# facebookresearch/D3GA

Hardware: AMD Instinct MI355X
Metric: fwd+bwd frames/sec @500k Gaussians 1920x1080 (higher is better)
Workload: dtype f32

## Files before the change

d3ga_amd/csrc/d3ga_internal.h:

```cpp
#pragma once
#include <hip/hip_runtime.h>
#include <stdint.h>

#include "../../include/d3ga.h"
#include "d3ga_math.h"

namespace d3ga {

constexpr int kBlock = 256;

int debug_knob(int key);

static inline int64_t align256(int64_t x) { return (x + 255) & ~int64_t(255); }

struct GeomBuf {
    float *depth;
    float4 *conic_o;
    float4 *rgb_invd;
    uint2 *rect;
    uint8_t *clamped;
    float *cov3D;
    float4 *xyh;
    float *dcol;
    int64_t dcol_stride;
};
static inline int64_t geom_bytes(int64_t P) {
    return align256(4 * P) + align256(16 * P) + align256(16 * P) + align256(8 * P) + align256(P) +
           align256(24 * P) + align256(16 * P) + align256(36 * P);
}
static inline GeomBuf carve_geom(void *base, int64_t P) {
    char *p = (char *)base;
    GeomBuf g;
    g.depth = (float *)p;     p += align256(4 * P);
    g.conic_o = (float4 *)p;  p += align256(16 * P);
    g.rgb_invd = (float4 *)p; p += align256(16 * P);
    g.rect = (uint2 *)p;      p += align256(8 * P);
    g.clamped = (uint8_t *)p; p += align256(P);
    g.cov3D = (float *)p;     p += align256(24 * P);
    g.xyh = (float4 *)p;      p += align256(16 * P);
    g.dcol = (float *)p;
    g.dcol_stride = P;
    return g;
}
__host__ __device__ static inline GeomBuf geom_view(const GeomBuf &g, int64_t P, int64_t v) {
    GeomBuf o = g;
    const int64_t d = v * P;
    o.depth += d; o.conic_o += d; o.rgb_invd += d; o.rect += d; o.clamped += d; o.cov3D += 6 * d; o.xyh += d; o.dcol += d;
    return o;
}

struct BinBuf {
    uint32_t *counters;
    uint32_t *tile_count;
    uint32_t *tile_start;
    uint32_t *tile_cursor;
    uint64_t *keys;
    uint32_t *point_list;
    uint32_t *big_tiles;
    uint32_t *huge_tiles;
    uint32_t *mid_tiles;
    uint32_t *tile_order;
};
static inline int64_t bin_bytes(int64_t tiles, int64_t dcap) {
    return 256 + align256(4 * tiles) + align256(4 * (tiles + 1)) + align256(4 * tiles) + align256(8 * dcap) +
           align256(4 * dcap) + 4 * align256(4 * tiles);
}
static inline BinBuf carve_bin(void *base, int64_t tiles, int64_t dcap) {
    char *p = (char *)base;
    BinBuf b;
    b.counters = (uint32_t *)p;    p += 256;
    b.tile_count = (uint32_t *)p;  p += align256(4 * tiles);
    b.tile_start = (uint32_t *)p;  p += align256(4 * (tiles + 1));
    b.tile_cursor = (uint32_t *)p; p += align256(4 * tiles);
    b.keys = (uint64_t *)p;        p += align256(8 * dcap);
    b.point_list = (uint32_t *)p;  p += align256(4 * dcap);
    b.big_tiles = (uint32_t *)p;   p += align256(4 * tiles);
    b.huge_tiles = (uint32_t *)p;  p += align256(4 * tiles);
    b.mid_tiles = (uint32_t *)p;   p += align256(4 * tiles);
    b.tile_order = (uint32_t *)p;
    return b;
}

struct ImgBuf {
    float *final_T;
    uint32_t *n_contrib;
    uint32_t *blk_count;
    uint2 *blk_list;
};
static inline int64_t img_bytes(int64_t W, int64_t H, int64_t tiles, int64_t dcap, int64_t views = 1) {
    return 2 * align256(4 * W * H * views) + align256(64 * tiles) + align256(128 * dcap);
}
static inline ImgBuf carve_img(void *base, int64_t W, int64_t H, int64_t tiles, int64_t views = 1) {
    ImgBuf i;
    char *p = (char *)base;
    i.final_T = (float *)p;        p += align256(4 * W * H * views);
    i.n_contrib = (uint32_t *)p;   p += align256(4 * W * H * views);
    i.blk_count = (uint32_t *)p;   p += align256(64 * tiles);
    i.blk_list = (uint2 *)p;
    return i;
}

constexpr int kWinTiles = 4096;

struct TileWindow {
    int x0, y0, w, h;
    __device__ __forceinline__ int area() const { return w * h; }
    __device__ __forceinline__ bool fits() const { return w * h <= kWinTiles; }
    __device__ __forceinline__ int tile_of(int k, int gx, float inv_w) const {
        const int r = (int)(((float)k + 0.5f) * inv_w);
        return (y0 + r) * gx + x0 + (k - r * w);
    }
};

#ifdef __HIPCC__
__device__ __forceinline__ TileWindow block_tile_window(int *s_box, bool visible, int rx0, int ry0, int rx1, int ry1) {
    if (threadIdx.x == 0) { s_box[0] = 0x7fffffff; s_box[1] = 0x7fffffff; s_box[2] = 0; s_box[3] = 0; }
    __syncthreads();
    int bx0 = visible ? rx0 : 0x7fffffff, by0 = visible ? ry0 : 0x7fffffff, bx1 = visible ? rx1 : 0, by1 = visible ? ry1 : 0;
#pragma unroll
    for (int off = 1; off < 64; off <<= 1) {
        bx0 = min(bx0, __shfl_xor(bx0, off)); by0 = min(by0, __shfl_xor(by0, off));
        bx1 = max(bx1, __shfl_xor(bx1, off)); by1 = max(by1, __shfl_xor(by1, off));
    }
    if ((threadIdx.x & 63) == 0 && bx1 > 0) {
        atomicMin(&s_box[0], bx0); atomicMin(&s_box[1], by0);
        atomicMax(&s_box[2], bx1); atomicMax(&s_box[3], by1);
    }
    __syncthreads();
    TileWindow win;
    win.x0 = s_box[0]; win.y0 = s_box[1];
    win.w = s_box[2] > s_box[0] ? s_box[2] - s_box[0] : 0;
    win.h = s_box[3] > s_box[1] ? s_box[3] - s_box[1] : 0;
    if (win.w == 0 || win.h == 0) { win.w = 0; win.h = 0; }
    return win;
}
#endif

static inline int tiles_x(int W) { return (W + kTile - 1) / kTile; }
static inline int tiles_y(int H) { return (H + kTile - 1) / kTile; }
static inline int n_views_of(const d3ga_raster_params *prm) { return prm->n_views > 1 ? prm->n_views : 1; }
static inline bool is_windowed(const d3ga_raster_params *prm) { return prm->tanfovx == D3GA_CAMERA_SLOT_WINDOWED; }
static inline int grid_x(const d3ga_raster_params *prm) { return tiles_x(prm->W) + (is_windowed(prm) ? 1 : 0); }
static inline int grid_y(const d3ga_raster_params *prm) { return tiles_y(prm->H) + (is_windowed(prm) ? 1 : 0); }
static inline int4 *win_table(void *binning, int64_t tiles, int64_t dcap) { return (int4 *)((char *)binning + bin_bytes(tiles, dcap)); }
static inline int64_t win_table_bytes(int64_t views) { return align256(16 * views); }

static inline int check_launch(hipStream_t s, int debug) {
    hipError_t e = hipGetLastError();
    if (e != hipSuccess) return (int)e;
    if (debug) {
        e = hipStreamSynchronize(s);
        if (e != hipSuccess) return (int)e;
    }
    return 0;
}

#define D3GA_TRY(expr)            \
    do {                          \
        int _st = (expr);         \
        if (_st != 0) return _st; \
    } while (0)
#define D3GA_HIP(expr)                          \
    do {                                        \
        hipError_t _e = (expr);                 \
        if (_e != hipSuccess) return (int)_e;   \
    } while (0)

#ifdef __HIPCC__
static __global__ void zero_words_kernel(uint32_t *__restrict__ p, size_t n) {
    for (size_t i = (size_t)blockIdx.x * blockDim.x + threadIdx.x; i < n; i += (size_t)gridDim.x * blockDim.x) p[i] = 0u;
}
static __global__ void zero_bytes_kernel(unsigned char *__restrict__ p, size_t n) {
    for (size_t i = (size_t)blockIdx.x * blockDim.x + threadIdx.x; i < n; i += (size_t)gridDim.x * blockDim.x) p[i] = 0;
}
static inline hipError_t zero_async(void *ptr, size_t bytes, hipStream_t s) {
    if (bytes == 0) return hipSuccess;
    if ((((uintptr_t)ptr | bytes) & 3) == 0) {
        const size_t n = bytes / 4;
        const size_t blocks = (n + 4 * kBlock - 1) / (4 * kBlock);
        hipLaunchKernelGGL(zero_words_kernel, dim3((unsigned)(blocks < 1 ? 1 : (blocks > 4096 ? 4096 : blocks))), dim3(kBlock), 0, s,
                           reinterpret_cast<uint32_t *>(ptr), n);
    } else {
        const size_t blocks = (bytes + kBlock - 1) / kBlock;
        hipLaunchKernelGGL(zero_bytes_kernel, dim3((unsigned)(blocks > 4096 ? 4096 : blocks)), dim3(kBlock), 0, s,
                           reinterpret_cast<unsigned char *>(ptr), bytes);
    }
    return hipGetLastError();
}
#endif

}
```

d3ga_amd/csrc/raster_api.hip:

```cpp
#include "d3ga_internal.h"

#include <atomic>

namespace d3ga {
static const int kKnobDefault[D3GA_KNOB_COUNT] = {
     32 | 128,  512,  2,  -1,  -1,
     1,  1,  0,  0};
static std::atomic<int> g_knob[D3GA_KNOB_COUNT] = {{32 | 128}, {512}, {2}, {-1}, {-1}, {1}, {1}, {0}, {0}};
int debug_knob(int key) { return (key >= 0 && key < D3GA_KNOB_COUNT) ? g_knob[key].load(std::memory_order_relaxed) : 0; }
}

using namespace d3ga;

extern "C" int d3ga_debug_set(int32_t key, int32_t value) {
    if (key < 0 || key >= D3GA_KNOB_COUNT) return D3GA_E_SIZE;
    g_knob[key].store(value == D3GA_KNOB_DEFAULT ? kKnobDefault[key] : value, std::memory_order_relaxed);
    return D3GA_OK;
}

extern "C" int d3ga_debug_defaults(int32_t *out, int32_t n) {
    if (!out) return D3GA_E_NULL;
    if (n < 2 + 2 * D3GA_KNOB_COUNT) return D3GA_E_SIZE;
#ifdef D3GA_SCAN_ABL
    out[0] = D3GA_SCAN_ABL;
#else
    out[0] = 0;
#endif
#ifdef D3GA_DIAG
    out[1] = 1;
#else
    out[1] = 0;
#endif
    for (int k = 0; k < D3GA_KNOB_COUNT; ++k) { out[2 + 2 * k] = kKnobDefault[k]; out[3 + 2 * k] = debug_knob(k); }
    return D3GA_OK;
}

extern "C" int d3ga_version(void) { return D3GA_VERSION; }

extern "C" const char *d3ga_status_string(int status) {
    switch (status) {
        case D3GA_OK: return "ok";
        case D3GA_E_NULL: return "required pointer is NULL";
        case D3GA_E_SIZE: return "negative or inconsistent size";
        case D3GA_E_CONFIG: return "unsupported argument combination";
        case D3GA_E_CAPACITY: return "scratch buffer too small";
        default: break;
    }
    if (status > 0) return hipGetErrorString((hipError_t)status);
    return "unknown status";
}

extern "C" int d3ga_raster_scratch_bytes_views(int32_t P, int32_t W, int32_t H, int32_t n_views, int64_t d_capacity,
                                               int32_t forward_only, int64_t sizes[3]) {
    if (!sizes) return D3GA_E_NULL;
    if (P < 0 || W <= 0 || H <= 0 || d_capacity < 0 || n_views < 0) return D3GA_E_SIZE;
    const int64_t k = n_views > 1 ? n_views : 1;
    if ((int64_t)tiles_y(H) * k > 65535 || (int64_t)P * k >= (1ll << 31)) return D3GA_E_SIZE;
    const int64_t tiles = (int64_t)tiles_x(W) * tiles_y(H) * k, cap = d_capacity > 0 ? d_capacity : 1;
    sizes[0] = geom_bytes(P > 0 ? P * k : 1);
    sizes[1] = bin_bytes(tiles, cap);
    sizes[2] = forward_only ? 2 * align256(4 * (int64_t)W * H * k) : img_bytes(W, H, tiles, cap, k);
    return D3GA_OK;
}

extern "C" int d3ga_raster_scratch_bytes_window(int32_t P, int32_t W, int32_t H, int32_t n_views, int64_t d_capacity,
                                                int32_t forward_only, int64_t sizes[3]) {
    if (!sizes) return D3GA_E_NULL;
    if (P < 0 || W <= 0 || H <= 0 || d_capacity < 0 || n_views < 0) return D3GA_E_SIZE;
    const int64_t k = n_views > 1 ? n_views : 1;
    const int64_t gx = tiles_x(W) + 1, gy = tiles_y(H) + 1;
    if (gy * k > 65535 || gx > 65535 || (int64_t)P * k >= (1ll << 31)) return D3GA_E_SIZE;
    const int64_t tiles = gx * gy * k, cap = d_capacity > 0 ? d_capacity : 1;
    sizes[0] = geom_bytes(P > 0 ? P * k : 1);
    sizes[1] = bin_bytes(tiles, cap) + win_table_bytes(k);
    sizes[2] = forward_only ? 2 * align256(4 * (int64_t)W * H * k) : img_bytes(W, H, tiles, cap, k);
    return D3GA_OK;
}

extern "C" int d3ga_raster_binning_layout_window(int32_t W, int32_t H, int32_t n_views, int64_t d_capacity, int64_t offsets[7]) {
    if (!offsets) return D3GA_E_NULL;
    if (W <= 0 || H <= 0 || d_capacity < 0 || n_views < 0) return D3GA_E_SIZE;
    const int64_t k = n_views > 1 ? n_views : 1, cap = d_capacity > 0 ? d_capacity : 1;
    const int64_t tiles = (int64_t)(tiles_x(W) + 1) * (tiles_y(H) + 1) * k;
    char *base = (char *)nullptr + 256;
    const BinBuf b = carve_bin(base, tiles, cap);
    offsets[0] = (char *)b.counters - base;
    offsets[1] = (char *)b.tile_count - base;
    offsets[2] = (char *)b.tile_start - base;
    offsets[3] = (char *)b.tile_cursor - base;
    offsets[4] = (char *)b.keys - base;
    offsets[5] = (char *)b.point_list - base;
    offsets[6] = (char *)win_table(base, tiles, cap) - base;
    return D3GA_OK;
}

extern "C" int d3ga_raster_scratch_bytes(int32_t P, int32_t W, int32_t H, int64_t d_capacity, int64_t sizes[3]) {
    return d3ga_raster_scratch_bytes_views(P, W, H, 1, d_capacity, 0, sizes);
}

extern "C" int64_t d3ga_raster_img_bytes(int32_t W, int32_t H, int64_t d_capacity, int32_t forward_only) {
    if (W <= 0 || H <= 0 || d_capacity < 0) return D3GA_E_SIZE;
    const int64_t tiles = (int64_t)tiles_x(W) * tiles_y(H);
    return forward_only ? 2 * align256(4 * (int64_t)W * H) : img_bytes(W, H, tiles, d_capacity > 0 ? d_capacity : 1);
}

extern "C" int d3ga_raster_binning_layout(int32_t W, int32_t H, int64_t d_capacity, int64_t offsets[6]) {
    if (!offsets) return D3GA_E_NULL;
    if (W <= 0 || H <= 0 || d_capacity < 0) return D3GA_E_SIZE;
    char *base = (char *)nullptr + 256;
    const BinBuf b = carve_bin(base, (int64_t)tiles_x(W) * tiles_y(H), d_capacity > 0 ? d_capacity : 1);
    offsets[0] = (char *)b.counters - base;
    offsets[1] = (char *)b.tile_count - base;
    offsets[2] = (char *)b.tile_start - base;
    offsets[3] = (char *)b.tile_cursor - base;
    offsets[4] = (char *)b.keys - base;
    offsets[5] = (char *)b.point_list - base;
    return D3GA_OK;
}

extern "C" int d3ga_raster_img_layout(int32_t W, int32_t H, int64_t offsets[2]) {
    if (!offsets) return D3GA_E_NULL;
    if (W <= 0 || H <= 0) return D3GA_E_SIZE;
    offsets[0] = 0;
    offsets[1] = align256(4 * (int64_t)W * H);
    return D3GA_OK;
}

extern "C" int d3ga_raster_img_layout_blocks(int32_t W, int32_t H, int64_t offsets[2]) {
    if (!offsets) return D3GA_E_NULL;
    if (W <= 0 || H <= 0) return D3GA_E_SIZE;
    const int64_t tiles = (int64_t)tiles_x(W) * tiles_y(H);
    char *base = (char *)nullptr + 256;
    const ImgBuf im = carve_img(base, W, H, tiles);
    offsets[0] = (char *)im.blk_count - base;
    offsets[1] = (char *)im.blk_list - base;
    return D3GA_OK;
}

extern "C" int d3ga_raster_forward(const d3ga_raster_params *prm, const float *means3D, const float *shs,
                                   const float *colors_precomp, const float *opacities, const float *scales,
                                   const float *rotations, const float *cov3D_precomp, const float *viewmatrix,
                                   const float *projmatrix, const float *campos, const float *bg, void *geom,
                                   void *binning, void *img, int64_t d_capacity, float *out_color, int32_t *radii,
                                   float *out_invdepth, d3ga_stream_t stream) {
    D3GA_TRY(d3ga_raster_preprocess(prm, means3D, shs, colors_precomp, opacities, scales, rotations, cov3D_precomp,
                                    viewmatrix, projmatrix, campos, geom, binning, d_capacity, radii, stream));
    D3GA_TRY(d3ga_raster_bin_sort(prm, geom, binning, d_capacity, stream));
    return d3ga_raster_composite_fwd(prm, bg, geom, binning, d_capacity, img, out_color, out_invdepth, stream);
}

extern "C" int d3ga_raster_backward(const d3ga_raster_params *prm, const float *means3D, const float *shs,
                                    const float *scales, const float *rotations, const float *cov3D_precomp,
                                    const float *viewmatrix, const float *projmatrix, const float *campos,
                                    const float *bg, const void *geom, const void *binning, int64_t d_capacity,
                                    const void *img, const float *dL_dpix, float *acc, float *dL_dmeans3D,
                                    float *dL_dmeans2D, float *dL_dopacity, float *dL_dsh, float *dL_dcolors,
                                    float *dL_dcov3D, float *dL_dscales, float *dL_drots, d3ga_stream_t stream) {
    if (prm && prm->P > 0 && acc && !prm->acc_self_clearing)
        D3GA_HIP(zero_async(acc, sizeof(float) * D3GA_ACC_STRIDE * (size_t)prm->P * (size_t)n_views_of(prm), (hipStream_t)stream));
    D3GA_TRY(d3ga_raster_composite_bwd(prm, bg, geom, binning, d_capacity, img, dL_dpix, acc, stream));
    return d3ga_raster_preprocess_bwd(prm, means3D, shs, scales, rotations, cov3D_precomp, viewmatrix, projmatrix,
                                      campos, geom, acc, dL_dmeans3D, dL_dmeans2D, dL_dopacity, dL_dsh, dL_dcolors,
                                      dL_dcov3D, dL_dscales, dL_drots, stream);
}

extern "C" int d3ga_raster_backward_l1(const d3ga_raster_params *prm, const float *means3D, const float *shs,
                                       const float *scales, const float *rotations, const float *cov3D_precomp,
                                       const float *viewmatrix, const float *projmatrix, const float *campos,
                                       const float *bg, const void *geom, const void *binning, int64_t d_capacity,
                                       const void *img, const float *image, const float *target, const void *target_cell,
                                       const float *g_loss, const float *dL_dpix, float *acc, float *dL_dmeans3D,
                                       float *dL_dmeans2D, float *dL_dopacity, float *dL_dsh, float *dL_dcolors,
                                       float *dL_dcov3D, float *dL_dscales, float *dL_drots, d3ga_stream_t stream) {
    if (prm && prm->P > 0 && acc && !prm->acc_self_clearing)
        D3GA_HIP(zero_async(acc, sizeof(float) * D3GA_ACC_STRIDE * (size_t)prm->P * (size_t)n_views_of(prm), (hipStream_t)stream));
    D3GA_TRY(d3ga_raster_composite_bwd_l1(prm, bg, geom, binning, d_capacity, img, image, target, target_cell, g_loss, dL_dpix,
                                          acc, stream));
    return d3ga_raster_preprocess_bwd(prm, means3D, shs, scales, rotations, cov3D_precomp, viewmatrix, projmatrix,
                                      campos, geom, acc, dL_dmeans3D, dL_dmeans2D, dL_dopacity, dL_dsh, dL_dcolors,
                                      dL_dcov3D, dL_dscales, dL_drots, stream);
}
```

d3ga_amd/csrc/raster_bin.hip:

```cpp
#include <atomic>

#include "composite_common.h"

namespace d3ga {

constexpr int kScanBlock = 1024;

__device__ __forceinline__ void tile_scan_body(int tiles, const uint32_t *__restrict__ count,
                                               uint32_t *__restrict__ start, uint32_t *__restrict__ cursor,
                                               uint32_t *__restrict__ counters, uint64_t dcap,
                                               uint32_t *__restrict__ big_tiles, uint32_t *__restrict__ huge_tiles,
                                               uint32_t *__restrict__ mid_tiles, uint32_t n_small, uint32_t n_mid,
                                               uint32_t n_large) {
    constexpr int kPer = 8, kChunk = kPer * kScanBlock;
    __shared__ uint32_t s_wave[2][kScanBlock / 64];
    __shared__ uint32_t s_max;
    const int tid = threadIdx.x, lane = tid & 63, wave = tid >> 6;
    if (tid == 0) s_max = 0;
    uint32_t carry = 0, mx = 0;
    int par = 0;
    for (int c0 = 0; c0 < tiles; c0 += kChunk, par ^= 1) {
        const int t0 = c0 + kPer * tid;
        uint32_t c[kPer];
        if (t0 + kPer <= tiles) {
            const uint4 lo = reinterpret_cast<const uint4 *>(count + t0)[0], hi = reinterpret_cast<const uint4 *>(count + t0)[1];
            c[0] = lo.x; c[1] = lo.y; c[2] = lo.z; c[3] = lo.w; c[4] = hi.x; c[5] = hi.y; c[6] = hi.z; c[7] = hi.w;
        } else {
#pragma unroll
            for (int k = 0; k < kPer; ++k) c[k] = t0 + k < tiles ? count[t0 + k] : 0u;
        }
        uint32_t sum = 0;
#pragma unroll
        for (int k = 0; k < kPer; ++k) { sum += c[k]; mx = max(mx, c[k]); }
        uint32_t incl = sum;
#pragma unroll
        for (int off = 1; off < 64; off <<= 1) {
            const uint32_t v = __shfl_up(incl, off);
            if (lane >= off) incl += v;
        }
        if (lane == 63) s_wave[par][wave] = incl;
        __syncthreads();
        uint32_t wbase = 0, total = 0;
#pragma unroll
        for (int w = 0; w < kScanBlock / 64; ++w) {
            const uint32_t v = s_wave[par][w];
            wbase += w < wave ? v : 0u;
            total += v;
        }
        uint32_t run = carry + wbase + incl - sum;
        uint32_t e[kPer];
        int cls[kPer];
#pragma unroll
        for (int k = 0; k < kPer; ++k) {
            e[k] = run;
            run += c[k];
            cls[k] = c[k] > n_large ? 2 : (c[k] > n_mid ? 1 : (c[k] > n_small ? 0 : -1));
        }
#pragma unroll
        for (int q = 0; q < 3; ++q) {
            uint32_t nq = 0;
#pragma unroll
            for (int k = 0; k < kPer; ++k) nq += cls[k] == q ? 1u : 0u;
            if (__ballot(nq != 0u) == 0ull) continue;
            uint32_t inq = nq;
#pragma unroll
            for (int off = 1; off < 64; off <<= 1) {
                const uint32_t v = __shfl_up(inq, off);
                if (lane >= off) inq += v;
            }
            const uint32_t tot = (uint32_t)__shfl((int)inq, 63);
            uint32_t base = 0;
            if (lane == 0) base = atomicAdd(&counters[q == 0 ? D3GA_CNT_MID : (q == 1 ? D3GA_CNT_BIG : D3GA_CNT_HUGE)], tot);
            uint32_t pos = (uint32_t)__shfl((int)base, 0) + inq - nq;
            uint32_t *list = q == 0 ? mid_tiles : (q == 1 ? big_tiles : huge_tiles);
#pragma unroll
            for (int k = 0; k < kPer; ++k)
                if (cls[k] == q) list[pos++] = (uint32_t)(t0 + k);
        }
        if (t0 + kPer <= tiles) {
            const uint4 lo = make_uint4(e[0], e[1], e[2], e[3]), hi = make_uint4(e[4], e[5], e[6], e[7]);
            reinterpret_cast<uint4 *>(start + t0)[0] = lo; reinterpret_cast<uint4 *>(start + t0)[1] = hi;
            reinterpret_cast<uint4 *>(cursor + t0)[0] = lo; reinterpret_cast<uint4 *>(cursor + t0)[1] = hi;
        } else {
#pragma unroll
            for (int k = 0; k < kPer; ++k)
                if (t0 + k < tiles) { start[t0 + k] = e[k]; cursor[t0 + k] = e[k]; }
        }
        carry += total;
    }
#pragma unroll
    for (int off = 1; off < 64; off <<= 1) mx = max(mx, (uint32_t)__shfl_xor((int)mx, off));
    if (lane == 0) atomicMax(&s_max, mx);
    __syncthreads();
    if (tid == 0) {
        start[tiles] = carry;
        counters[D3GA_CNT_D] = carry;
        counters[D3GA_CNT_OVERFLOW] = (uint64_t)carry > dcap ? 1u : 0u;
        counters[D3GA_CNT_MAXTILE] = s_max;
    }
}

__device__ __forceinline__ void tile_order_body(int tiles, const uint32_t *__restrict__ count,
                                                uint32_t *__restrict__ order, uint32_t *__restrict__ counters) {
    __shared__ uint32_t s_hist[256];
    __shared__ uint32_t s_zero;
    const int tid = threadIdx.x, lane = tid & 63;
    constexpr int kPer = 8;
    if (tid < 256) s_hist[tid] = 0;
    if (tid == 0) s_zero = 0;
    __syncthreads();
    auto bucket = [](uint32_t c) { return 254u - min(c >> 4, 254u); };
    for (int c0 = 0; c0 < tiles; c0 += kPer * kScanBlock) {
        uint32_t c[kPer];
#pragma unroll
        for (int k = 0; k < kPer; ++k) {
            const int t = c0 + k * kScanBlock + tid;
            c[k] = t < tiles ? count[t] : 0xffffffffu;
        }
#pragma unroll
        for (int k = 0; k < kPer; ++k) {
            const bool zero = c[k] == 0u;
            const unsigned long long zm = __ballot(zero);
            if (lane == 0 && zm) atomicAdd(&s_zero, (uint32_t)__popcll(zm));
            if (c[k] != 0u && c[k] != 0xffffffffu) atomicAdd(&s_hist[bucket(c[k])], 1u);
        }
        if (c0 + kPer * kScanBlock < tiles) continue;
        __syncthreads();
        if (tid < 64) {
            uint32_t v[4], sum = 0;
#pragma unroll
            for (int k = 0; k < 4; ++k) { v[k] = (4 * tid + k < 255) ? s_hist[4 * tid + k] : 0u; sum += v[k]; }
            uint32_t incl = sum;
#pragma unroll
            for (int off = 1; off < 64; off <<= 1) {
                const uint32_t u = __shfl_up(incl, off);
                if (tid >= off) incl += u;
            }
            uint32_t run = incl - sum;
#pragma unroll
            for (int k = 0; k < 4; ++k) { s_hist[4 * tid + k] = run; run += v[k]; }
        }
        __syncthreads();
        if (tid == 0) {
            s_zero = s_hist[255];
            counters[D3GA_CNT_HEAVY] = s_hist[255] <= 4096u ? (s_hist[255] + 9u) / 10u : 0u;
        }
        __syncthreads();
        for (int c1 = 0; c1 < tiles; c1 += kPer * kScanBlock) {
            if (c0 != 0) {
#pragma unroll
                for (int k = 0; k < kPer; ++k) {
                    const int t = c1 + k * kScanBlock + tid;
                    c[k] = t < tiles ? count[t] : 0xffffffffu;
                }
            }
#pragma unroll
            for (int k = 0; k < kPer; ++k) {
                const int t = c1 + k * kScanBlock + tid;
                const bool zero = c[k] == 0u;
                const unsigned long long zm = __ballot(zero);
                uint32_t zbase = 0;
                if (lane == 0 && zm) zbase = atomicAdd(&s_zero, (uint32_t)__popcll(zm));
                zbase = (uint32_t)__shfl((int)zbase, 0);
                if (zero) order[zbase + (uint32_t)__popcll(zm & ((1ull << lane) - 1ull))] = (uint32_t)t;
                if (c[k] != 0u && c[k] != 0xffffffffu) order[atomicAdd(&s_hist[bucket(c[k])], 1u)] = (uint32_t)t;
            }
        }
    }
}

__global__ __launch_bounds__(kScanBlock) void tile_scan_order_kernel(int tiles, const uint32_t *__restrict__ count,
                                                                     uint32_t *__restrict__ start,
                                                                     uint32_t *__restrict__ cursor,
                                                                     uint32_t *__restrict__ counters, uint64_t dcap,
                                                                     uint32_t *__restrict__ big_tiles,
                                                                     uint32_t *__restrict__ huge_tiles,
                                                                     uint32_t *__restrict__ mid_tiles, uint32_t n_small,
                                                                     uint32_t n_mid, uint32_t n_large,
                                                                     uint32_t *__restrict__ order) {
    if (blockIdx.x == 0) tile_scan_body(tiles, count, start, cursor, counters, dcap, big_tiles, huge_tiles, mid_tiles, n_small, n_mid, n_large);
    else tile_order_body(tiles, count, order, counters);
}

__global__ __launch_bounds__(kBlock) void tile_scatter_kernel(int P, int gx, const uint2 *__restrict__ rect,
                                                              const float *__restrict__ depth,
                                                              uint32_t *__restrict__ cursor, uint64_t *__restrict__ keys,
                                                              uint64_t dcap) {
    __shared__ int s_box[4];
    __shared__ uint32_t s_cnt[kWinTiles];
    const int tid = threadIdx.x;
    const int i = blockIdx.x * kBlock + tid;
    int x0 = 0, y0 = 0, x1 = 0, y1 = 0;
    uint64_t key = 0;
    if (i < P) {
        const uint2 rc = rect[i];
        x0 = rc.x & 0xffffu; y0 = rc.x >> 16; x1 = rc.y & 0xffffu; y1 = rc.y >> 16;
        key = ((uint64_t)__float_as_uint(depth[i]) << 32) | (uint32_t)i;
    }
    const bool visible = x1 > x0 && y1 > y0;
    const TileWindow win = block_tile_window(s_box, visible, x0, y0, x1, y1);
    const int area = win.area();
    if (area == 0) return;
    if (win.fits()) {
        for (int k = tid; k < area; k += kBlock) s_cnt[k] = 0;
        __syncthreads();
        if (visible)
            for (int ty = y0; ty < y1; ++ty)
                for (int tx = x0; tx < x1; ++tx) atomicAdd(&s_cnt[(ty - win.y0) * win.w + (tx - win.x0)], 1u);
        __syncthreads();
        const float inv_w = 1.0f / (float)win.w;
        for (int k = tid; k < area; k += kBlock) {
            const uint32_t c = s_cnt[k];
            if (c) s_cnt[k] = atomicAdd(&cursor[win.tile_of(k, gx, inv_w)], c);
        }
        __syncthreads();
        if (visible)
            for (int ty = y0; ty < y1; ++ty)
                for (int tx = x0; tx < x1; ++tx) {
                    const int l = (ty - win.y0) * win.w + (tx - win.x0);
                    const uint32_t pos = atomicAdd(&s_cnt[l], 1u);
                    if (pos < dcap) keys[pos] = key;
                }
    } else if (visible) {
        for (int ty = y0; ty < y1; ++ty)
            for (int tx = x0; tx < x1; ++tx) {
                const uint32_t pos = atomicAdd(&cursor[ty * gx + tx], 1u);
                if (pos < dcap) keys[pos] = key;
            }
    }
}

template <typename KeyPtr>
__device__ __forceinline__ void bitonic_sort(KeyPtr k, int n, int tid, int nthreads) {
    int n2 = 1;
    while (n2 < n) n2 <<= 1;
    const int half = n2 >> 1;
    for (int size = 2, lsz = 1; size <= n2; size <<= 1, ++lsz) {
        const int hs = size >> 1;
        for (int i = tid; i < half; i += nthreads) {
            const int blk = i >> (lsz - 1), off = i & (hs - 1);
            const int lo = (blk << lsz) + off, hi = (blk << lsz) + size - 1 - off;
            if (hi < n) {
                const uint64_t a = k[lo], b = k[hi];
                if (b < a) { k[lo] = b; k[hi] = a; }
            }
        }
        __syncthreads();
        for (int j = hs >> 1, lj = lsz - 2; j >= 1; j >>= 1, --lj) {
            for (int i = tid; i < half; i += nthreads) {
                const int blk = i >> lj, off = i & (j - 1);
                const int lo = (blk << (lj + 1)) + off, hi = lo + j;
                if (hi < n) {
                    const uint64_t a = k[lo], b = k[hi];
                    if (b < a) { k[lo] = b; k[hi] = a; }
                }
            }
            __syncthreads();
        }
    }
}

template <int BLOCK, int CAP>
__device__ __forceinline__ void sort_one_tile_bucket(uint64_t *s_key, uint32_t *s_bin, uint32_t *s_red, int tile,
                                                     const uint32_t *__restrict__ start, const uint64_t *__restrict__ keys,
                                                     uint32_t *__restrict__ point_list, uint64_t dcap) {
    static_assert(CAP == 8 * BLOCK, "eight keys / eight counters per thread");
    constexpr int NW = BLOCK / 64;
    const uint64_t b64 = min((uint64_t)start[tile], dcap), e64 = min((uint64_t)start[tile + 1], dcap);
    const int n = min((int)(e64 - b64), CAP);
    const int tid = threadIdx.x, lane = tid & 63, wave = tid >> 6;
    uint64_t r[8];
    uint32_t lo = 0xffffffffu, hi = 0u;
#pragma unroll
    for (int k = 0; k < 8; ++k) {
        const int i = tid + k * BLOCK;
        r[k] = i < n ? keys[b64 + i] : ~0ull;
    }
#pragma unroll
    for (int k = 0; k < 8; ++k) {
        const int i = tid + k * BLOCK;
        if (i < n) { const uint32_t d = (uint32_t)(r[k] >> 32); lo = min(lo, d); hi = max(hi, d); }
    }
#pragma unroll
    for (int off = 1; off < 64; off <<= 1) {
        lo = min(lo, (uint32_t)__shfl_xor((int)lo, off));
        hi = max(hi, (uint32_t)__shfl_xor((int)hi, off));
    }
    if (lane == 0) { s_red[wave] = lo; s_red[NW + wave] = hi; }
#pragma unroll
    for (int k = 0; k < 8; ++k) s_bin[tid + k * BLOCK] = 0u;
    __syncthreads();
#pragma unroll
    for (int w = 0; w < NW; ++w) { lo = min(lo, s_red[w]); hi = max(hi, s_red[NW + w]); }
    const uint32_t range = hi - lo;
    int sh = 32 - __clz((int)(range | 1u)) - (31 - __clz(CAP));
    if (range & 0x80000000u) sh = 32 - (31 - __clz(CAP));
    sh = max(sh, 0);
    uint32_t bucket[8], slot[8];
#pragma unroll
    for (int k = 0; k < 8; ++k) {
        const int i = tid + k * BLOCK;
        bucket[k] = ((uint32_t)(r[k] >> 32) - lo) >> sh;
        slot[k] = 0u;
        if (i < n) slot[k] = atomicAdd(&s_bin[bucket[k]], 1u);
    }
    __syncthreads();
    {
        uint32_t c[8], sum = 0;
#pragma unroll
        for (int k = 0; k < 8; ++k) { c[k] = s_bin[8 * tid + k]; sum += c[k]; }
        uint32_t incl = sum;
#pragma unroll
        for (int off = 1; off < 64; off <<= 1) {
            const uint32_t u = (uint32_t)__shfl_up((int)incl, off);
            if (lane >= off) incl += u;
        }
        if (lane == 63) s_red[wave] = incl;
        __syncthreads();
        uint32_t run = incl - sum;
#pragma unroll
        for (int w = 0; w < NW; ++w) if (w < wave) run += s_red[w];
#pragma unroll
        for (int k = 0; k < 8; ++k) { s_bin[8 * tid + k] = run; run += c[k]; }
        if (tid == BLOCK - 1) s_bin[CAP] = run;
    }
    __syncthreads();
#pragma unroll
    for (int k = 0; k < 8; ++k) {
        const int i = tid + k * BLOCK;
        if (i < n) s_key[s_bin[bucket[k]] + slot[k]] = r[k];
    }
    __syncthreads();
#pragma unroll
    for (int k = 0; k < 8; ++k) {
        const int i = tid + k * BLOCK;
        if (i < n) {
            const uint32_t b0 = s_bin[bucket[k]], b1 = s_bin[bucket[k] + 1];
            uint32_t less = 0;
            for (uint32_t p = b0; p < b1; ++p) less += s_key[p] < r[k] ? 1u : 0u;
            point_list[b64 + b0 + less] = (uint32_t)r[k];
        }
    }
}

template <int BLOCK, int CAP>
__device__ __forceinline__ bool sort_huge_tile_bucket(uint64_t *s_key, uint32_t *s_bin, uint32_t *s_cur, uint32_t *s_red, int tile,
                                                      const uint32_t *__restrict__ start, const uint64_t *__restrict__ keys,
                                                      uint32_t *__restrict__ point_list, uint64_t dcap) {
    static_assert(CAP == 8 * BLOCK, "eight counters per thread");
    constexpr int NW = BLOCK / 64;
    const uint64_t b64 = min((uint64_t)start[tile], dcap), e64 = min((uint64_t)start[tile + 1], dcap);
    const int n = (int)(e64 - b64);
    const int tid = threadIdx.x, lane = tid & 63, wave = tid >> 6;
    uint32_t lo = 0xffffffffu, hi = 0u;
    for (int i = tid; i < n; i += BLOCK) { const uint32_t d = (uint32_t)(keys[b64 + i] >> 32); lo = min(lo, d); hi = max(hi, d); }
#pragma unroll
    for (int off = 1; off < 64; off <<= 1) {
        lo = min(lo, (uint32_t)__shfl_xor((int)lo, off));
        hi = max(hi, (uint32_t)__shfl_xor((int)hi, off));
    }
    __syncthreads();
    if (lane == 0) { s_red[wave] = lo; s_red[NW + wave] = hi; }
#pragma unroll
    for (int k = 0; k < 8; ++k) s_bin[tid + k * BLOCK] = 0u;
    __syncthreads();
#pragma unroll
    for (int w = 0; w < NW; ++w) { lo = min(lo, s_red[w]); hi = max(hi, s_red[NW + w]); }
    const uint32_t range = hi - lo;
    const int sh = max(32 - __clz((int)(range | 1u)) - (31 - __clz(CAP)), 0);
    for (int i = tid; i < n; i += BLOCK) atomicAdd(&s_bin[((uint32_t)(keys[b64 + i] >> 32) - lo) >> sh], 1u);
    __syncthreads();
    uint32_t cmax = 0;
    {
        uint32_t c[8], sum = 0;
#pragma unroll
        for (int k = 0; k < 8; ++k) { c[k] = s_bin[8 * tid + k]; sum += c[k]; cmax = max(cmax, c[k]); }
        uint32_t incl = sum;
#pragma unroll
        for (int off = 1; off < 64; off <<= 1) {
            const uint32_t u = (uint32_t)__shfl_up((int)incl, off);
            if (lane >= off) incl += u;
            cmax = max(cmax, (uint32_t)__shfl_xor((int)cmax, off));
        }
        __syncthreads();
        if (lane == 63) { s_red[wave] = incl; s_red[NW + wave] = cmax; }
        __syncthreads();
        uint32_t run = incl - sum;
#pragma unroll
        for (int w = 0; w < NW; ++w) { if (w < wave) run += s_red[w]; cmax = max(cmax, s_red[NW + w]); }
#pragma unroll
        for (int k = 0; k < 8; ++k) { s_bin[8 * tid + k] = run; run += c[k]; }
        if (tid == BLOCK - 1) s_bin[CAP] = run;
    }
    __syncthreads();
    if (cmax > (uint32_t)CAP) return false;
    for (int segA = 0; segA < CAP;) {
        if (tid == 0) {
            const uint32_t limit = s_bin[segA] + (uint32_t)CAP;
            int a = segA + 1, b = CAP;
            while (a < b) { const int m = (a + b + 1) >> 1; if (s_bin[m] <= limit) a = m; else b = m - 1; }
            s_red[0] = (uint32_t)a;
        }
#pragma unroll
        for (int k = 0; k < 8; ++k) s_cur[tid + k * BLOCK] = 0u;
        __syncthreads();
        const int segB = (int)s_red[0];
        const uint32_t baseA = s_bin[segA], m = s_bin[segB] - baseA;
        if (m) {
            for (int i = tid; i < n; i += BLOCK) {
                const uint64_t key = keys[b64 + i];
                const uint32_t b = ((uint32_t)(key >> 32) - lo) >> sh;
                if (b >= (uint32_t)segA && b < (uint32_t)segB) s_key[s_bin[b] - baseA + atomicAdd(&s_cur[b], 1u)] = key;
            }
            __syncthreads();
            for (uint32_t i = tid; i < m; i += BLOCK) {
                const uint64_t key = s_key[i];
                const uint32_t b = ((uint32_t)(key >> 32) - lo) >> sh;
                const uint32_t b0 = s_bin[b] - baseA, b1 = s_bin[b + 1] - baseA;
                uint32_t less = 0;
                for (uint32_t p = b0; p < b1; ++p) less += s_key[p] < key ? 1u : 0u;
                point_list[b64 + baseA + b0 + less] = (uint32_t)key;
            }
        }
        __syncthreads();
        segA = segB;
    }
    return true;
}

template <int BLOCK, int CAP>
__global__ __launch_bounds__(BLOCK) void tile_sort_lds_kernel(const uint32_t *__restrict__ start,
                                                              const uint64_t *__restrict__ keys,
                                                              uint32_t *__restrict__ point_list, uint64_t dcap,
                                                              const uint32_t *__restrict__ order, int tiles) {
    __shared__ uint64_t s_key[CAP];
    __shared__ __attribute__((aligned(8))) uint32_t s_bin[CAP + 1];
    __shared__ uint32_t s_red[2 * (BLOCK / 64)];
    for (int rank = blockIdx.x; rank < tiles; rank += gridDim.x) {
        const int tile = (int)order[rank];
        const uint32_t n = start[tile + 1] - start[tile];
        if (n == 0) return;
        if (n <= (uint32_t)CAP) sort_one_tile_bucket<BLOCK, CAP>(s_key, s_bin, s_red, tile, start, keys, point_list, dcap);
        __syncthreads();
    }
}

template <int BLOCK, int CAP>
__global__ __launch_bounds__(BLOCK) void tile_sort_lds_list_kernel(const uint32_t *__restrict__ start,
                                                                   const uint64_t *__restrict__ keys,
                                                                   uint32_t *__restrict__ point_list, uint64_t dcap,
                                                                   const uint32_t *__restrict__ list,
                                                                   const uint32_t *__restrict__ list_count,
                                                                   uint64_t *__restrict__ keys_rw,
                                                                   const uint32_t *__restrict__ huge_list,
                                                                   const uint32_t *__restrict__ huge_count,
                                                                   const uint32_t *__restrict__ list2,
                                                                   const uint32_t *__restrict__ list2_count) {
    extern __shared__ __attribute__((aligned(16))) uint64_t s_key_dyn[];
    uint32_t *s_bin = reinterpret_cast<uint32_t *>(s_key_dyn + CAP);
    uint32_t *s_red = s_bin + CAP + 1;
    uint32_t *s_cur = s_red + 2 * (BLOCK / 64) + 2;
    const uint32_t count = *list_count;
    for (uint32_t v = blockIdx.x; v < count; v += gridDim.x) {
        __syncthreads();
        sort_one_tile_bucket<BLOCK, CAP>(s_key_dyn, s_bin, s_red, (int)list[v], start, keys, point_list, dcap);
    }
    if (list2) {
        const uint32_t count2 = *list2_count;
        for (uint32_t v = gridDim.x - 1u - blockIdx.x; v < count2; v += gridDim.x) {
            __syncthreads();
            sort_one_tile_bucket<BLOCK, CAP>(s_key_dyn, s_bin, s_red, (int)list2[v], start, keys, point_list, dcap);
        }
    }
    if (huge_list) {
        const uint32_t hcount = *huge_count;
        const int tid = threadIdx.x;
        for (uint32_t k = blockIdx.x; k < hcount; k += gridDim.x) {
            const int tile = (int)huge_list[k];
            const uint64_t b64 = min((uint64_t)start[tile], dcap), e64 = min((uint64_t)start[tile + 1], dcap);
            const int n = (int)(e64 - b64);
            __syncthreads();
            if (!sort_huge_tile_bucket<BLOCK, CAP>(s_key_dyn, s_bin, s_cur, s_red, tile, start, keys, point_list, dcap)) {
                bitonic_sort(keys_rw + b64, n, tid, BLOCK);
                for (int i = tid; i < n; i += BLOCK) point_list[b64 + i] = (uint32_t)keys_rw[b64 + i];
            }
        }
    }
}

}

using namespace d3ga;

constexpr int kSortSmall = 2048;
constexpr int kSortMid = 4096;
constexpr int kSortLarge = 8192;
static inline size_t sort_lds_bytes(int cap, int block, bool huge = false) {
    return (size_t)cap * 8 + ((size_t)cap + 1 + 2 * (block / 64) + 2 + (huge ? cap : 0)) * 4 + 16;
}


extern "C" int d3ga_raster_bin_sort(const d3ga_raster_params *prm, void *geom, void *binning, int64_t d_capacity,
                                    d3ga_stream_t stream) {
    if (!prm || !geom || !binning) return D3GA_E_NULL;
    if (prm->P < 0 || prm->W <= 0 || prm->H <= 0 || d_capacity < 0) return D3GA_E_SIZE;
    hipStream_t s = (hipStream_t)stream;
    const int views = n_views_of(prm);
    const int gx = grid_x(prm);
    const int tiles = gx * grid_y(prm) * views;
    const int64_t P = (int64_t)prm->P * views;
    BinBuf bin = carve_bin(binning, tiles, d_capacity);
    GeomBuf g = carve_geom(geom, P);
    hipLaunchKernelGGL(tile_scan_order_kernel, dim3(2), dim3(kScanBlock), 0, s, tiles, bin.tile_count, bin.tile_start,
                       bin.tile_cursor, bin.counters, (uint64_t)d_capacity, bin.big_tiles, bin.huge_tiles, bin.mid_tiles,
                       (uint32_t)kSortSmall, (uint32_t)kSortMid, (uint32_t)kSortLarge, bin.tile_order);
    D3GA_TRY(check_launch(s, prm->debug));
    if (P == 0 || d_capacity == 0) return D3GA_OK;
    hipLaunchKernelGGL(tile_scatter_kernel, dim3((unsigned)((P + kBlock - 1) / kBlock)), dim3(kBlock), 0, s, (int)P, gx, g.rect,
                       g.depth, bin.tile_cursor, bin.keys, (uint64_t)d_capacity);
    D3GA_TRY(check_launch(s, prm->debug));
    {
        static std::atomic<int> resident[64] = {};
        int dev = 0;
        D3GA_HIP(hipGetDevice(&dev));
        int want = (dev >= 0 && dev < 64) ? resident[dev].load(std::memory_order_relaxed) : 0;
        if (want == 0) {
            int per_cu = 0, cus = 0;
            if (hipOccupancyMaxActiveBlocksPerMultiprocessor(&per_cu, (const void *)tile_sort_lds_kernel<256, kSortSmall>, 256, 0) != hipSuccess || per_cu < 1) per_cu = 4;
            if (hipDeviceGetAttribute(&cus, hipDeviceAttributeMultiprocessorCount, dev) != hipSuccess || cus < 1) cus = 256;
            want = per_cu * cus;
            if (dev >= 0 && dev < 64) resident[dev].store(want, std::memory_order_relaxed);
        }
        hipLaunchKernelGGL((tile_sort_lds_kernel<256, kSortSmall>), dim3(tiles < want ? tiles : want), dim3(256), 0, s, bin.tile_start,
                           bin.keys, bin.point_list, (uint64_t)d_capacity, (const uint32_t *)bin.tile_order, tiles);
    }
    D3GA_TRY(check_launch(s, prm->debug));
    {
        static std::atomic<bool> attr_set[64] = {};
        int dev = 0;
        D3GA_HIP(hipGetDevice(&dev));
        if (dev >= 0 && dev < 64 && !attr_set[dev].load(std::memory_order_relaxed)) {
            D3GA_HIP(hipFuncSetAttribute((const void *)tile_sort_lds_list_kernel<1024, kSortLarge>,
                                         hipFuncAttributeMaxDynamicSharedMemorySize, (int)sort_lds_bytes(kSortLarge, 1024, true)));
            attr_set[dev].store(true, std::memory_order_relaxed);
        }
    }
    const int lgrid = tiles < 256 ? tiles : 256, mgrid = tiles < 768 ? tiles : 768;
    const int merge_knob = debug_knob(D3GA_KNOB_SORT_MERGE);
    const bool merged = merge_knob >= 0 ? merge_knob != 0 : d_capacity / (tiles > 0 ? tiles : 1) < 320;
#define D3GA_LAUNCH_LIST_SORT(BLOCKV, CAPV, GRID, HUGE, LIST, CNT, KEYS_RW, HLIST, HCNT, LIST2, CNT2)                              \
    hipLaunchKernelGGL((tile_sort_lds_list_kernel<BLOCKV, CAPV>), dim3(GRID), dim3(BLOCKV), sort_lds_bytes(CAPV, BLOCKV, HUGE), s, \
                       bin.tile_start, bin.keys, bin.point_list, (uint64_t)d_capacity, LIST, CNT, KEYS_RW, HLIST, HCNT, LIST2, CNT2)
    const uint32_t *const nil = nullptr;
    if (!merged) {
        D3GA_LAUNCH_LIST_SORT(512, kSortMid, mgrid, false, bin.mid_tiles, bin.counters + D3GA_CNT_MID, (uint64_t *)nullptr, nil, nil, nil, nil);
        D3GA_TRY(check_launch(s, prm->debug));
    }
    const uint32_t *l2 = merged ? (const uint32_t *)bin.mid_tiles : nil, *c2 = merged ? (const uint32_t *)(bin.counters + D3GA_CNT_MID) : nil;
    D3GA_LAUNCH_LIST_SORT(1024, kSortLarge, lgrid, true, bin.big_tiles, bin.counters + D3GA_CNT_BIG, bin.keys,
                          (const uint32_t *)bin.huge_tiles, (const uint32_t *)(bin.counters + D3GA_CNT_HUGE), l2, c2);
#undef D3GA_LAUNCH_LIST_SORT
    return check_launch(s, prm->debug);
}
```

d3ga_amd/csrc/raster_pre.hip:

```cpp
#include "composite_common.h"
#include "raster_pre_body.h"

namespace d3ga {

constexpr int kShRow = 52;
constexpr int kShSlab = 64 * kShRow;
constexpr size_t kShLdsBytes = (size_t)(kBlock / 64) * kShSlab * sizeof(float);

__host__ __device__ __forceinline__ bool sh_staged(int M) { return M > 0 && (3 * M) % 4 == 0 && 3 * M <= 48; }

__device__ __forceinline__ void sh_slab_load(float *slab, const float *__restrict__ src, int rows, int M3, int lane) {
    const int nvec = rows * M3 / 4;
    for (int v = lane; v < nvec; v += 64) {
        const float4 x = reinterpret_cast<const float4 *>(src)[v];
        const int e = 4 * v, r = e / M3, c = e - r * M3;
        *reinterpret_cast<float4 *>(slab + r * kShRow + c) = x;
    }
}
__device__ __forceinline__ void sh_slab_store(const float *slab, float *__restrict__ dst, int rows, int M3, int lane) {
    const int nvec = rows * M3 / 4;
    for (int v = lane; v < nvec; v += 64) {
        const int e = 4 * v, r = e / M3, c = e - r * M3;
        reinterpret_cast<float4 *>(dst)[v] = *reinterpret_cast<const float4 *>(slab + r * kShRow + c);
    }
}

template <int ROWS>
struct ShRegs { float4 v[ROWS * 12 / 64]; };
template <int ROWS>
__device__ __forceinline__ ShRegs<ROWS> sh_rows48_load(const float *__restrict__ src, int lane) {
    ShRegs<ROWS> r;
#pragma unroll
    for (int k = 0; k < ROWS * 12 / 64; ++k) r.v[k] = reinterpret_cast<const float4 *>(src)[lane + 64 * k];
    return r;
}
template <int ROWS>
__device__ __forceinline__ void sh_rows48_to_slab(float *slab, const ShRegs<ROWS> &r, int lane) {
#pragma unroll
    for (int k = 0; k < ROWS * 12 / 64; ++k) {
        const int e = 4 * (lane + 64 * k), row = e / 48, c = e - row * 48;
        *reinterpret_cast<float4 *>(slab + row * kShRow + c) = r.v[k];
    }
}
template <int ROWS>
__device__ __forceinline__ void sh_rows48_store(const float *slab, float *__restrict__ dst, int lane) {
#pragma unroll
    for (int k = 0; k < ROWS * 12 / 64; ++k) {
        const int e = 4 * (lane + 64 * k), row = e / 48, c = e - row * 48;
        reinterpret_cast<float4 *>(dst)[lane + 64 * k] = *reinterpret_cast<const float4 *>(slab + row * kShRow + c);
    }
}

constexpr int kShPassRows = 32;
constexpr int kShHalfSlab = kShPassRows * kShRow;
constexpr size_t kShHalfLdsBytes = (size_t)(kBlock / 64) * kShHalfSlab * sizeof(float);

template <bool WANT_J>
__device__ __forceinline__ void staged_sh_colour(const d3ga_raster_params &prm, const float *__restrict__ means3D,
                                                 const float *__restrict__ shs, const float *__restrict__ campos,
                                                 float *s_sh, float acc[3], ShColJ &cj) {
    const int tid = threadIdx.x, lane = tid & 63, wave = tid >> 6;
    const int i = blockIdx.x * kBlock + tid;
    const int M3 = 3 * prm.M;
    float *slab = s_sh + wave * kShHalfSlab;
    const int row0 = blockIdx.x * kBlock + wave * 64;
    const int rows = min(64, prm.P - row0);
    const int nb = (prm.sh_degree + 1) * (prm.sh_degree + 1);
    float B[16];
    float dx = 0.f, dy = 0.f, dz = 1.f;
    if (WANT_J && i < prm.P) sh_view_dir(means3D, i, campos, dx, dy, dz);
    auto eval = [&](const float *row) __attribute__((always_inline)) {
        if (WANT_J) cj = sh_accumulate_jacobian(B, dx, dy, dz, row, nb, cj);
        else sh_accumulate(B, row, 0, 16, nb, acc);
    };
    if (M3 == 48 && rows == 64) {
        const float *src = shs + (size_t)48 * row0;
        const ShRegs<kShPassRows> h0 = sh_rows48_load<kShPassRows>(src, lane);
        const ShRegs<kShPassRows> h1 = sh_rows48_load<kShPassRows>(src + 48 * kShPassRows, lane);
        sh_view_basis(prm, means3D, i, campos, B);
        __builtin_amdgcn_wave_barrier();
        sh_rows48_to_slab<kShPassRows>(slab, h0, lane);
        __builtin_amdgcn_wave_barrier();
        if (lane / kShPassRows == 0) eval(slab + (lane % kShPassRows) * kShRow);
        __builtin_amdgcn_wave_barrier();
        sh_rows48_to_slab<kShPassRows>(slab, h1, lane);
        __builtin_amdgcn_wave_barrier();
        if (lane / kShPassRows == 1) eval(slab + (lane % kShPassRows) * kShRow);
        return;
    }
    if (i < prm.P) sh_view_basis(prm, means3D, i, campos, B);
    for (int h = 0; h < 2; ++h) {
        const int r = min(kShPassRows, rows - kShPassRows * h);
        __builtin_amdgcn_wave_barrier();
        if (r > 0) sh_slab_load(slab, shs + (size_t)M3 * (row0 + kShPassRows * h), r, M3, lane);
        __builtin_amdgcn_wave_barrier();
        if (i < prm.P && lane / kShPassRows == h) eval(slab + (lane % kShPassRows) * kShRow);
    }
}

struct TileRect { bool visible; int r0, r1, r2, r3; };
__device__ __forceinline__ TileRect write_geom_records(const GeomBuf &geom, int i, const PreOut &o, bool keep_cov, int tile_row0,
                                                       int32_t *__restrict__ radii, bool want_j, const ShColJ &cj) {
    const Splat &sp = o.sp;
    if (keep_cov) {
#pragma unroll
        for (int k = 0; k < 6; ++k) geom.cov3D[6 * (size_t)i + k] = o.c6[k];
    }
    radii[i] = sp.radius;
    geom.depth[i] = sp.depth;
    geom.rect[i] = sp.visible ? make_uint2((uint32_t)sp.rect[0] | ((uint32_t)(sp.rect[1] + tile_row0) << 16),
                                           (uint32_t)sp.rect[2] | ((uint32_t)(sp.rect[3] + tile_row0) << 16))
                              : make_uint2(0u, 0u);
    geom.conic_o[i] = make_float4(sp.conic[0], sp.conic[1], sp.conic[2], o.opacity);
    {
        const SplatCull sc = splat_cull(sp.conic[0], sp.conic[1], sp.conic[2], o.opacity);
        geom.xyh[i] = make_float4(sp.px, sp.py, sp.visible ? sc.hx : -1.0f, sc.hy);
    }
    geom.rgb_invd[i] = make_float4(o.rgb[0], o.rgb[1], o.rgb[2], sp.visible ? 1.0f / sp.depth : 0.f);
    geom.clamped[i] = o.clampmask;
    if (want_j) dcol_store(geom.dcol, geom.dcol_stride, i, cj);
    return TileRect{sp.visible, sp.rect[0], sp.rect[1] + tile_row0, sp.rect[2], sp.rect[3] + tile_row0};
}

__device__ __forceinline__ PreOut window_clip(PreOut o, int x0, int y0, int gx, int gy) {
    Splat &sp = o.sp;
    const int r0 = max(sp.rect[0], x0) - x0, r1 = max(sp.rect[1], y0) - y0;
    const int r2 = min(sp.rect[2], x0 + gx) - x0, r3 = min(sp.rect[3], y0 + gy) - y0;
    if (sp.visible && r2 > r0 && r3 > r1) { sp.rect[0] = r0; sp.rect[1] = r1; sp.rect[2] = r2; sp.rect[3] = r3; }
    else { sp.visible = false; sp.rect[0] = sp.rect[1] = sp.rect[2] = sp.rect[3] = 0; }
    return o;
}
__global__ void window_table_kernel(d3ga_raster_params prm, const float *__restrict__ campos, int views, int4 *__restrict__ table) {
    const int v = blockIdx.x * blockDim.x + threadIdx.x;
    if (v >= views) return;
    const ViewCam c = view_cam(prm, nullptr, nullptr, campos + (size_t)D3GA_CAMERA_SLOT_WINDOWED_FLOATS * v, true);
    table[v] = make_int4(c.ox, c.oy, c.W, c.H);
}

__device__ __forceinline__ void tile_histogram(int *s_box, uint32_t *s_cnt, const TileRect &t, int gx, uint32_t *__restrict__ tile_count,
                                               uint32_t *__restrict__ counters) {
    const int tid = threadIdx.x;
    const TileWindow win = block_tile_window(s_box, t.visible, t.r0, t.r1, t.r2, t.r3);
    const int nvis = __syncthreads_count(t.visible);
    if (tid == 0 && nvis) atomicAdd(&counters[D3GA_CNT_VISIBLE], (uint32_t)nvis);
    const int area = win.area();
    if (area == 0) return;
    if (win.fits()) {
        for (int k = tid; k < area; k += kBlock) s_cnt[k] = 0;
        __syncthreads();
        if (t.visible)
            for (int ty = t.r1; ty < t.r3; ++ty)
                for (int tx = t.r0; tx < t.r2; ++tx) atomicAdd(&s_cnt[(ty - win.y0) * win.w + (tx - win.x0)], 1u);
        __syncthreads();
        const float inv_w = 1.0f / (float)win.w;
        for (int k = tid; k < area; k += kBlock) {
            const uint32_t c = s_cnt[k];
            if (c) atomicAdd(&tile_count[win.tile_of(k, gx, inv_w)], c);
        }
    } else if (t.visible) {
        for (int ty = t.r1; ty < t.r3; ++ty)
            for (int tx = t.r0; tx < t.r2; ++tx) atomicAdd(&tile_count[ty * gx + tx], 1u);
    }
}

template <bool WIN>
__device__ __forceinline__ TileRect preprocess_view(const d3ga_raster_params &prm, const ViewCam &cam, int i, const float *means3D,
                                                    const float *sh_row, bool staged, const ShColJ &cj, bool pre, const float (&pc6)[6],
                                                    float pop, const float *colors_precomp, const float *opacities, const float *scales,
                                                    const float *rotations, const float *cov3D_precomp, const GeomBuf &geom,
                                                    int tile_row0, int32_t *radii, bool want_j, int gx, int gy) {
    PreLoaded pl;
    pl.has_sh = staged; pl.has_c6 = pre;
    pl.sh[0] = cj.a0; pl.sh[1] = cj.a1; pl.sh[2] = cj.a2;
#pragma unroll
    for (int k = 0; k < 6; ++k) pl.c6[k] = pc6[k];
    pl.op = pop;
    PreOut o = preprocess_one(prm, cam, i, means3D, sh_row, colors_precomp, opacities, scales, rotations, cov3D_precomp, pl);
    if constexpr (WIN) o = window_clip(o, cam.ox / kTile, cam.oy / kTile, gx, gy);
    return write_geom_records(geom, i, o, !cov3D_precomp, tile_row0, radii, want_j, cj);
}

template <bool WANT_J, bool WIN>
__global__ __launch_bounds__(kBlock) void preprocess_kernel(
    d3ga_raster_params prm, const float *__restrict__ means3D, const float *__restrict__ shs,
    const float *__restrict__ colors_precomp, const float *__restrict__ opacities, const float *__restrict__ scales,
    const float *__restrict__ rotations, const float *__restrict__ cov3D_precomp, const float *__restrict__ viewmatrix,
    const float *__restrict__ projmatrix, const float *__restrict__ campos, GeomBuf geom,
    uint32_t *__restrict__ tile_count, uint32_t *__restrict__ counters, int32_t *__restrict__ radii,
    int tile_row0 ) {
    const ViewCam cam = view_cam(prm, viewmatrix, projmatrix, campos, WIN);
    const int gx = (prm.W + kTile - 1) / kTile + (WIN ? 1 : 0), gy = (prm.H + kTile - 1) / kTile + 1;
    extern __shared__ __attribute__((aligned(16))) char smem[];
    __shared__ int s_box[4];
    float *s_sh = reinterpret_cast<float *>(smem);
    uint32_t *s_cnt = reinterpret_cast<uint32_t *>(smem);
    const int tid = threadIdx.x;
    const int i = blockIdx.x * kBlock + tid;
    const int M3 = 3 * prm.M;
    const bool staged = shs != nullptr && sh_staged(prm.M);
    float pc6[6] = {0.f, 0.f, 0.f, 0.f, 0.f, 0.f}, pop = 0.f;
    const bool pre = staged && cov3D_precomp != nullptr;
    if (pre && i < prm.P) {
#pragma unroll
        for (int k = 0; k < 6; ++k) pc6[k] = cov3D_precomp[6 * (size_t)i + k];
        pop = opacities[i];
    }
    ShColJ cj = {0.f, 0.f, 0.f, 0.f, 0.f, 0.f, 0.f, 0.f, 0.f, 0.f, 0.f, 0.f};
    float acc[3] = {0.f, 0.f, 0.f};
    if (staged) {
        staged_sh_colour<WANT_J>(prm, means3D, shs, campos, s_sh, acc, cj);
        if (!WANT_J) { cj.a0 = acc[0]; cj.a1 = acc[1]; cj.a2 = acc[2]; }
        __syncthreads();
    }
    TileRect tr = {false, 0, 0, 0, 0};
    if (i < prm.P) {
        tr = staged ? preprocess_view<WIN>(prm, cam, i, means3D, nullptr, true, cj, pre, pc6, pop, colors_precomp, opacities, scales,
                                           rotations, cov3D_precomp, geom, tile_row0, radii, WANT_J, gx, gy)
                    : preprocess_view<WIN>(prm, cam, i, means3D, shs ? shs + (size_t)M3 * i : nullptr, false, cj, false, pc6, pop,
                                           colors_precomp, opacities, scales, rotations, cov3D_precomp, geom, tile_row0, radii,
                                           WANT_J, gx, gy);
    }
    tile_histogram(s_box, s_cnt, tr, gx, tile_count, counters);
}

template <bool WANT_J, int KV>
__device__ __forceinline__ void staged_sh_colour_views(const d3ga_raster_params &prm, const float *__restrict__ means3D, size_t pv,
                                                       const float *__restrict__ shs, const ViewCams<KV> &cams, float *s_sh,
                                                       ShColJ (&cj)[KV]) {
    const int tid = threadIdx.x, lane = tid & 63, wave = tid >> 6;
    const int i = blockIdx.x * kBlock + tid;
    const int M3 = 3 * prm.M;
    float *slab = s_sh + wave * kShHalfSlab;
    const int row0 = blockIdx.x * kBlock + wave * 64;
    const int rows = min(64, prm.P - row0);
    const int nb = (prm.sh_degree + 1) * (prm.sh_degree + 1);
    auto eval = [&](const float *row) __attribute__((always_inline)) {
#pragma unroll
        for (int v = 0; v < KV; ++v) {
            float B[16];
            const float *mv = means3D + 3 * pv * v;
            if (WANT_J) {
                float dx, dy, dz;
                sh_view_dir(mv, i, cams.cp[v], dx, dy, dz);
                sh_basis(prm.sh_degree, dx, dy, dz, B);
                cj[v] = sh_accumulate_jacobian(B, dx, dy, dz, row, nb, cj[v]);
            } else {
                sh_view_basis(prm, mv, i, cams.cp[v], B);
                float acc[3] = {cj[v].a0, cj[v].a1, cj[v].a2};
                sh_accumulate(B, row, 0, 16, nb, acc);
                cj[v].a0 = acc[0]; cj[v].a1 = acc[1]; cj[v].a2 = acc[2];
            }
        }
    };
    if (M3 == 48 && rows == 64) {
        const float *src = shs + (size_t)48 * row0;
        const ShRegs<kShPassRows> h0 = sh_rows48_load<kShPassRows>(src, lane);
        const ShRegs<kShPassRows> h1 = sh_rows48_load<kShPassRows>(src + 48 * kShPassRows, lane);
        __builtin_amdgcn_wave_barrier();
        sh_rows48_to_slab<kShPassRows>(slab, h0, lane);
        __builtin_amdgcn_wave_barrier();
        if (lane / kShPassRows == 0) eval(slab + (lane % kShPassRows) * kShRow);
        __builtin_amdgcn_wave_barrier();
        sh_rows48_to_slab<kShPassRows>(slab, h1, lane);
        __builtin_amdgcn_wave_barrier();
        if (lane / kShPassRows == 1) eval(slab + (lane % kShPassRows) * kShRow);
        return;
    }
    for (int h = 0; h < 2; ++h) {
        const int r = min(kShPassRows, rows - kShPassRows * h);
        __builtin_amdgcn_wave_barrier();
        if (r > 0) sh_slab_load(slab, shs + (size_t)M3 * (row0 + kShPassRows * h), r, M3, lane);
        __builtin_amdgcn_wave_barrier();
        if (i < prm.P && lane / kShPassRows == h) eval(slab + (lane % kShPassRows) * kShRow);
    }
}

template <bool WANT_J, int KV>
__global__ __launch_bounds__(kBlock) void preprocess_views_kernel(
    d3ga_raster_params prm, const float *__restrict__ means3D, const float *__restrict__ shs,
    const float *__restrict__ colors_precomp, const float *__restrict__ opacities, const float *__restrict__ scales,
    const float *__restrict__ rotations, const float *__restrict__ cov3D_precomp, ViewCams<KV> cams, GeomBuf geom ,
    uint32_t *__restrict__ tile_count, uint32_t *__restrict__ counters, int32_t *__restrict__ radii ,
    int tile_row0, int gyv, size_t pv ) {
    extern __shared__ __attribute__((aligned(16))) char smem[];
    __shared__ int s_box[4];
    float *s_sh = reinterpret_cast<float *>(smem);
    uint32_t *s_cnt = reinterpret_cast<uint32_t *>(smem);
    const int tid = threadIdx.x;
    const int i = blockIdx.x * kBlock + tid;
    float pc6[6] = {0.f, 0.f, 0.f, 0.f, 0.f, 0.f}, pop = 0.f;
    const bool pre = cov3D_precomp != nullptr && pv == 0;
    if (pre && i < prm.P) {
#pragma unroll
        for (int k = 0; k < 6; ++k) pc6[k] = cov3D_precomp[6 * (size_t)i + k];
        pop = opacities[i];
    }
    ShColJ cj[KV];
#pragma unroll
    for (int v = 0; v < KV; ++v) cj[v] = ShColJ{0.f, 0.f, 0.f, 0.f, 0.f, 0.f, 0.f, 0.f, 0.f, 0.f, 0.f, 0.f};
    staged_sh_colour_views<WANT_J, KV>(prm, means3D, pv, shs, cams, s_sh, cj);
    const int gx = (prm.W + kTile - 1) / kTile;
#pragma unroll
    for (int v = 0; v < KV; ++v) {
        __syncthreads();
        TileRect tr = {false, 0, 0, 0, 0};
        if (i < prm.P) {
            const size_t og = pv * v;
            tr = preprocess_view<false>(prm, view_cam(prm, cams.vm[v], cams.pm[v], cams.cp[v], false), i, means3D + 3 * og, nullptr, true,
                                        cj[v], pre, pc6, pop, colors_precomp, opacities, scales ? scales + 3 * og : nullptr,
                                        rotations ? rotations + 4 * og : nullptr, cov3D_precomp ? cov3D_precomp + 6 * og : nullptr,
                                        geom_view(geom, prm.P, v), tile_row0 + v * gyv, radii + (size_t)prm.P * v, WANT_J, gx, 0);
        }
        tile_histogram(s_box, s_cnt, tr, gx, tile_count, counters);
    }
}

template <bool WANT_J>
__global__ __launch_bounds__(kBlock) void recolor_kernel(d3ga_raster_params prm, const float *__restrict__ means3D,
                                                         const float *__restrict__ shs,
                                                         const float *__restrict__ colors_precomp,
                                                         const float *__restrict__ campos, GeomBuf src, GeomBuf dst) {
    extern __shared__ __attribute__((aligned(16))) char smem[];
    float *s_sh = reinterpret_cast<float *>(smem);
    const int i = blockIdx.x * kBlock + threadIdx.x;
    const int M3 = 3 * prm.M;
    const bool staged = shs != nullptr && sh_staged(prm.M);
    ShColJ cj = {0.f, 0.f, 0.f, 0.f, 0.f, 0.f, 0.f, 0.f, 0.f, 0.f, 0.f, 0.f};
    float acc[3] = {0.f, 0.f, 0.f};
    if (staged) staged_sh_colour<WANT_J>(prm, means3D, shs, campos, s_sh, acc, cj);
    if (i >= prm.P) return;
    if (WANT_J) {
        acc[0] = cj.a0; acc[1] = cj.a1; acc[2] = cj.a2;
        dcol_store(dst.dcol, dst.dcol_stride, i, cj);
    }
    const uint2 rc = src.rect[i];
    const bool visible = rect_visible(rc.x, rc.y);
    const float depth = src.depth[i];
    dst.depth[i] = depth;
    dst.conic_o[i] = src.conic_o[i];
    dst.xyh[i] = src.xyh[i];
    dst.rect[i] = rc;
#pragma unroll
    for (int k = 0; k < 6; ++k) dst.cov3D[6 * (size_t)i + k] = src.cov3D[6 * (size_t)i + k];
    float rgb[3] = {0.f, 0.f, 0.f};
    uint8_t mask = 0;
    if (visible) {
        if (colors_precomp) {
            rgb[0] = colors_precomp[3 * (size_t)i]; rgb[1] = colors_precomp[3 * (size_t)i + 1];
            rgb[2] = colors_precomp[3 * (size_t)i + 2];
        } else {
            if (!staged) {
                float B[16];
                sh_view_basis(prm, means3D, i, campos, B);
                sh_accumulate(B, shs + (size_t)M3 * i, 0, 16, (prm.sh_degree + 1) * (prm.sh_degree + 1), acc);
            }
#pragma unroll
            for (int c = 0; c < 3; ++c) {
                const float v = acc[c] + 0.5f;
                if (v < 0.f) mask |= (uint8_t)(1u << c);
                rgb[c] = fmaxf(v, 0.f);
            }
        }
    }
    dst.rgb_invd[i] = make_float4(rgb[0], rgb[1], rgb[2], visible ? 1.0f / depth : 0.f);
    dst.clamped[i] = mask;
}

__device__ __forceinline__ ViewRecs view_recs(const GeomBuf &g, const float *acc) {
    return ViewRecs{reinterpret_cast<const uint32_t *>(g.rect), acc, g.clamped, reinterpret_cast<const float *>(g.conic_o), g.dcol,
                    g.dcol_stride};
}

template <bool WIN>
__global__ __launch_bounds__(kBlock) void preprocess_bwd_kernel(
    d3ga_raster_params prm, const float *__restrict__ means3D, const float *__restrict__ shs,
    const float *__restrict__ scales, const float *__restrict__ rotations, const float *__restrict__ viewmatrix,
    const float *__restrict__ projmatrix, const float *__restrict__ campos, GeomBuf geom,
    const float *__restrict__ acc, float *__restrict__ dL_dmeans3D, float *__restrict__ dL_dmeans2D,
    float *__restrict__ dL_dopacity, float *__restrict__ dL_dsh, float *__restrict__ dL_dcolors,
    float *__restrict__ dL_dcov3D, float *__restrict__ dL_dscales, float *__restrict__ dL_drots,
    const float *__restrict__ cov3D_precomp, int accum ) {
    const ViewCam cam = view_cam(prm, viewmatrix, projmatrix, campos, WIN);
    extern __shared__ __attribute__((aligned(16))) char smem[];
    float *s_sh = reinterpret_cast<float *>(smem);
    const int tid = threadIdx.x, lane = tid & 63, wave = tid >> 6;
    const int i = blockIdx.x * kBlock + tid;
    const int M3 = 3 * prm.M;
    const bool staged = shs != nullptr && sh_staged(prm.M);
    const int row0 = blockIdx.x * kBlock + wave * 64;
    const int rows = min(64, prm.P - row0);
    float *slab = s_sh + wave * kShSlab;
    const bool full48 = M3 == 48 && rows == 64;
    uint2 rc = make_uint2(0u, 0u);
    AccRec ar;
    float c6[6] = {0.f, 0.f, 0.f, 0.f, 0.f, 0.f};
    uint8_t clampmask = 0;
    float act_opacity = 0.f;
    if (i < prm.P) {
        rc = geom.rect[i];
        ar = acc_load(acc, i, prm.acc_self_clearing);
#pragma unroll
        for (int k = 0; k < 6; ++k) c6[k] = (cov3D_precomp ? cov3D_precomp : geom.cov3D)[6 * (size_t)i + k];
        clampmask = geom.clamped[i];
        act_opacity = geom.conic_o[i].w;
    }
    const bool have_j = staged && !prm.forward_only;
    ShColJ jd = {0.f, 0.f, 0.f, 0.f, 0.f, 0.f, 0.f, 0.f, 0.f, 0.f, 0.f, 0.f};
    if (have_j && i < prm.P) jd = dcol_load(geom.dcol, geom.dcol_stride, i);
    if (staged && !have_j) {
        if (full48) sh_rows48_to_slab<64>(slab, sh_rows48_load<64>(shs + (size_t)48 * row0, lane), lane);
        else if (rows > 0) sh_slab_load(slab, shs + (size_t)M3 * row0, rows, M3, lane);
        __builtin_amdgcn_wave_barrier();
    }
    if (i < prm.P) {
        const bool visible = rect_visible(rc.x, rc.y);
        if (!visible) {
#pragma unroll
            for (int k = 0; k < 12; ++k) ar.a[k] = 0.f;
#pragma unroll
            for (int k = 0; k < 6; ++k) c6[k] = 0.f;
            act_opacity = 0.f;
        }
        if (staged)
            preprocess_bwd_one(prm, cam, i, visible, means3D, slab + lane * kShRow, scales, rotations, c6, clampmask, ar.a, dL_dmeans3D,
                               dL_dmeans2D, dL_dopacity, dL_dsh ? slab + lane * kShRow : nullptr, dL_dcolors, dL_dcov3D, dL_dscales,
                               dL_drots, act_opacity, have_j, jd, accum);
        else
            preprocess_bwd_one(prm, cam, i, visible, means3D, shs ? shs + (size_t)M3 * i : nullptr, scales, rotations, c6, clampmask,
                               ar.a, dL_dmeans3D, dL_dmeans2D, dL_dopacity, dL_dsh ? dL_dsh + (size_t)M3 * i : nullptr, dL_dcolors,
                               dL_dcov3D, dL_dscales, dL_drots, act_opacity, false, ShColJ(), accum);
    }
    if (staged && dL_dsh) {
        __builtin_amdgcn_wave_barrier();
        if (full48) sh_rows48_store<64>(slab, dL_dsh + (size_t)48 * row0, lane);
        else if (rows > 0) sh_slab_store(slab, dL_dsh + (size_t)M3 * row0, rows, M3, lane);
    }
}

constexpr int kMaxGroup = 8;
template <bool WIN>
__global__ __launch_bounds__(kBlock) void preprocess_bwd_views_kernel(
    d3ga_raster_params prm, int kv, const float *__restrict__ means3D, bool sh_path, const float *__restrict__ scales,
    const float *__restrict__ rotations, const float *__restrict__ cov3D_precomp, ViewCams<kMaxGroup> cams, GeomBuf geom ,
    const float *__restrict__ acc , float *__restrict__ dL_dmeans3D, float *__restrict__ dL_dmeans2D ,
    float *__restrict__ dL_dopacity, float *__restrict__ dL_dsh, float *__restrict__ dL_dcolors, float *__restrict__ dL_dcov3D,
    float *__restrict__ dL_dscales, float *__restrict__ dL_drots, bool accum,
    size_t pv ,
    bool pva ) {
    extern __shared__ __attribute__((aligned(16))) char smem[];
    float *s_sh = reinterpret_cast<float *>(smem);
    const int tid = threadIdx.x, lane = tid & 63, wave = tid >> 6;
    const int i = blockIdx.x * kBlock + tid;
    const int M3 = 3 * prm.M;
    const int row0 = blockIdx.x * kBlock + wave * 64;
    const int rows = min(64, prm.P - row0);
    float *slab = s_sh + wave * kShSlab;
    if (i < prm.P)
        preprocess_bwd_views_one(prm, i, kv, WIN, cams, view_recs(geom, acc), means3D, cov3D_precomp ? cov3D_precomp : geom.cov3D,
                                 scales, rotations, sh_path, pv, pva, accum, dL_dmeans3D, dL_dmeans2D, dL_dopacity, dL_dcolors,
                                 dL_dcov3D, dL_dscales, dL_drots, sh_path && dL_dsh ? slab + lane * kShRow : nullptr);
    if (sh_path && dL_dsh) {
        __builtin_amdgcn_wave_barrier();
        if (accum) {
            const int nvec = rows > 0 ? rows * M3 / 4 : 0;
            float4 *dst = reinterpret_cast<float4 *>(dL_dsh + (size_t)M3 * row0);
            for (int v = lane; v < nvec; v += 64) {
                const int e = 4 * v, r = e / M3, c = e - r * M3;
                const float4 x = *reinterpret_cast<const float4 *>(slab + r * kShRow + c);
                float4 y = dst[v];
                y.x += x.x; y.y += x.y; y.z += x.z; y.w += x.w;
                dst[v] = y;
            }
        } else if (M3 == 48 && rows == 64) sh_rows48_store<64>(slab, dL_dsh + (size_t)48 * row0, lane);
        else if (rows > 0) sh_slab_store(slab, dL_dsh + (size_t)M3 * row0, rows, M3, lane);
    }
}

__global__ __launch_bounds__(kBlock) void sh_grad_from_views_kernel(
    int P, int M, int sh_degree, int n_views, const float *__restrict__ means3D, int64_t means_stride ,
    const float *__restrict__ g_views, int64_t g_stride, const float *__restrict__ campos_views, int64_t campos_stride, float scale,
    float *__restrict__ dL_dsh) {
    extern __shared__ __attribute__((aligned(16))) char smem[];
    float *s_sh = reinterpret_cast<float *>(smem);
    const int tid = threadIdx.x, lane = tid & 63, wave = tid >> 6;
    const int i = blockIdx.x * kBlock + tid;
    const int M3 = 3 * M;
    const bool staged = sh_staged(M);
    const int row0 = blockIdx.x * kBlock + wave * 64;
    const int rows = min(64, P - row0);
    float *slab = s_sh + wave * kShSlab;
    if (i < P) {
        float out[48];
#pragma unroll
        for (int k = 0; k < 48; ++k) out[k] = 0.f;
        const int nb = (sh_degree + 1) * (sh_degree + 1);
        for (int v = 0; v < n_views; ++v) {
            const float *g = g_views + v * g_stride + 3 * (size_t)i;
            const float g0 = g[0], g1 = g[1], g2 = g[2];
            if (g0 == 0.f && g1 == 0.f && g2 == 0.f) continue;
            const V3 mean = ld3(means3D + v * means_stride, i);
            const float *cp = campos_views + v * campos_stride;
            const V3 d0 = mean - v3(cp[0], cp[1], cp[2]);
            const float inv = 1.0f / sqrtf(dot(d0, d0));
            float B[16];
            sh_basis(sh_degree, d0.x * inv, d0.y * inv, d0.z * inv, B);
#pragma unroll
            for (int k = 0; k < 16; ++k)
                if (k < nb) {
                    out[3 * k] += B[k] * g0; out[3 * k + 1] += B[k] * g1; out[3 * k + 2] += B[k] * g2;
                }
        }
        float *row = staged ? slab + lane * kShRow : nullptr;
#pragma unroll
        for (int k = 0; k < 48; ++k)
            if (k < M3) {
                if (staged) row[k] = out[k] * scale;
                else dL_dsh[(size_t)M3 * i + k] = out[k] * scale;
            }
    }
    if (staged) {
        __syncthreads();
        if (rows > 0) sh_slab_store(slab, dL_dsh + (size_t)M3 * row0, rows, M3, lane);
    }
}

__global__ __launch_bounds__(kBlock) void mark_visible_kernel(int P, const float *__restrict__ means3D,
                                                              const float *__restrict__ viewmatrix,
                                                              uint8_t *__restrict__ visible) {
    const int i = blockIdx.x * kBlock + threadIdx.x;
    if (i >= P) return;
    visible[i] = xform_point(viewmatrix, ld3(means3D, i)).z > kNear ? 1 : 0;
}

}

using namespace d3ga;

static int validate(const d3ga_raster_params *prm) {
    if (!prm) return D3GA_E_NULL;
    if (prm->P < 0 || prm->W <= 0 || prm->H <= 0 || prm->M < 0 || prm->M > 16) return D3GA_E_SIZE;
    if (prm->sh_degree < 0 || prm->sh_degree > 3) return D3GA_E_CONFIG;
    if (prm->n_views < 0) return D3GA_E_SIZE;
    if (grid_x(prm) > 65535 || (int64_t)grid_y(prm) * n_views_of(prm) > 65535) return D3GA_E_SIZE;
    if ((int64_t)prm->P * n_views_of(prm) >= (1ll << 31)) return D3GA_E_SIZE;
    return D3GA_OK;
}

static bool staged(const d3ga_raster_params *prm, const float *shs) { return shs != nullptr && sh_staged(prm->M); }
static bool leaves_dcol(const d3ga_raster_params *prm, const float *shs) { return staged(prm, shs) && !prm->forward_only; }
static size_t lds_bytes(bool staged, size_t slabs, size_t floor = 0) { return staged && slabs > floor ? slabs : floor; }
static int cam_stride(const d3ga_raster_params *prm) {
    return prm->tanfovx > 0.f ? 3 : (is_windowed(prm) ? D3GA_CAMERA_SLOT_WINDOWED_FLOATS : 5);
}
template <int K>
static ViewCams<K> view_cams(const float *vm, const float *pm, const float *cp, int stride, int v0, int kv) {
    ViewCams<K> c;
    for (int q = 0; q < K; ++q) {
        const int v = v0 + (q < kv ? q : 0);
        c.vm[q] = vm + 16 * (size_t)v; c.pm[q] = pm + 16 * (size_t)v; c.cp[q] = cp + (size_t)stride * v;
    }
    return c;
}
template <class T>
static T *at(T *p, size_t n, size_t r) { return p ? p + n * r : nullptr; }

extern "C" int d3ga_raster_preprocess(const d3ga_raster_params *prm, const float *means3D, const float *shs,
                                      const float *colors_precomp, const float *opacities, const float *scales,
                                      const float *rotations, const float *cov3D_precomp, const float *viewmatrix,
                                      const float *projmatrix, const float *campos, void *geom, void *binning,
                                      int64_t d_capacity, int32_t *radii, d3ga_stream_t stream) {
    D3GA_TRY(validate(prm));
    if (!geom || !binning || !viewmatrix || !projmatrix || !campos) return D3GA_E_NULL;
    if (d_capacity < 0) return D3GA_E_SIZE;
    hipStream_t s = (hipStream_t)stream;
    const int views = n_views_of(prm), gyv = grid_y(prm);
    const int64_t tiles = (int64_t)grid_x(prm) * gyv * views;
    const bool wnd = is_windowed(prm);
    BinBuf bin = carve_bin(binning, tiles, d_capacity);
    D3GA_HIP(zero_async(bin.counters, 256 + align256(4 * tiles), s));
    if (wnd) hipLaunchKernelGGL(window_table_kernel, dim3((views + 63) / 64), dim3(64), 0, s, *prm, campos, views, win_table(binning, tiles, d_capacity));
    if (prm->P == 0) return D3GA_OK;
    if ((shs != nullptr) == (colors_precomp != nullptr)) return D3GA_E_CONFIG;
    const bool pva = views > 1 && prm->per_view_appearance;
    if (pva && shs) return D3GA_E_CONFIG;
    const bool sr = scales != nullptr && rotations != nullptr;
    if (sr == (cov3D_precomp != nullptr)) return D3GA_E_CONFIG;
    if (shs && (prm->sh_degree + 1) * (prm->sh_degree + 1) > prm->M) return D3GA_E_CONFIG;
    if (!means3D || !opacities || !radii) return D3GA_E_NULL;
    const GeomBuf g = carve_geom(geom, (int64_t)prm->P * views);
    const size_t lds = lds_bytes(staged(prm, shs), kShHalfLdsBytes, (size_t)kWinTiles * 4);
    const bool want_j = leaves_dcol(prm, shs);
    const int cs = cam_stride(prm);
    const size_t pv = (views > 1 && prm->per_view_geometry) ? (size_t)prm->P : 0;
    const size_t pa = pva ? (size_t)prm->P : 0;
    const dim3 grid((prm->P + kBlock - 1) / kBlock), block(kBlock);
    int v0 = 0;
    const bool grouped = views > 1 && !pva && !wnd && staged(prm, shs);
    auto launch_group = [&](auto kv) {
        constexpr int KV = decltype(kv)::value;
        const size_t og = pv * v0;
        hipLaunchKernelGGL((want_j ? preprocess_views_kernel<true, KV> : preprocess_views_kernel<false, KV>), grid, block, lds, s, *prm,
                           at(means3D, 3, og), shs, colors_precomp, opacities, at(scales, 3, og), at(rotations, 4, og),
                           at(cov3D_precomp, 6, og), view_cams<KV>(viewmatrix, projmatrix, campos, cs, v0, KV), geom_view(g, prm->P, v0),
                           bin.tile_count, bin.counters, radii + (size_t)prm->P * v0, v0 * gyv, gyv, pv);
        v0 += KV;
    };
    while (grouped && views - v0 >= 2) {
        const int left = views - v0;
        if (left >= 4 && left != 5) launch_group(std::integral_constant<int, 4>());
        else if (left == 3 || left == 5) launch_group(std::integral_constant<int, 3>());
        else launch_group(std::integral_constant<int, 2>());
    }
    const auto kernel = want_j ? (wnd ? preprocess_kernel<true, true> : preprocess_kernel<true, false>)
                               : (wnd ? preprocess_kernel<false, true> : preprocess_kernel<false, false>);
    for (int v = v0; v < views; ++v) {
        const ViewCams<1> c = view_cams<1>(viewmatrix, projmatrix, campos, cs, v, 1);
        const size_t og = pv * v, oa = pa * v;
        hipLaunchKernelGGL(kernel, grid, block, lds, s, *prm, at(means3D, 3, og), shs, at(colors_precomp, 3, oa), opacities + oa,
                           at(scales, 3, og), at(rotations, 4, og), at(cov3D_precomp, 6, og), c.vm[0], c.pm[0], c.cp[0],
                           geom_view(g, prm->P, v), bin.tile_count, bin.counters, radii + (size_t)prm->P * v, v * gyv);
    }
    return check_launch(s, prm->debug & 0xff);
}

extern "C" int d3ga_raster_recolor(const d3ga_raster_params *prm, const float *means3D, const float *shs,
                                   const float *colors_precomp, const float *campos, const void *geom_src,
                                   void *geom_dst, d3ga_stream_t stream) {
    D3GA_TRY(validate(prm));
    if (n_views_of(prm) > 1 || is_windowed(prm)) return D3GA_E_CONFIG;
    if (prm->P == 0) return D3GA_OK;
    if (!geom_src || !geom_dst || geom_src == geom_dst) return D3GA_E_NULL;
    if ((shs != nullptr) == (colors_precomp != nullptr)) return D3GA_E_CONFIG;
    if (shs && (!means3D || !campos)) return D3GA_E_NULL;
    if (shs && (prm->sh_degree + 1) * (prm->sh_degree + 1) > prm->M) return D3GA_E_CONFIG;
    hipStream_t s = (hipStream_t)stream;
    const GeomBuf src = carve_geom(const_cast<void *>(geom_src), prm->P), dst = carve_geom(geom_dst, prm->P);
    hipLaunchKernelGGL(leaves_dcol(prm, shs) ? recolor_kernel<true> : recolor_kernel<false>, dim3((prm->P + kBlock - 1) / kBlock),
                       dim3(kBlock), lds_bytes(staged(prm, shs), kShHalfLdsBytes), s, *prm, means3D, shs, colors_precomp, campos, src, dst);
    return check_launch(s, prm->debug & 0xff);
}

extern "C" int d3ga_raster_preprocess_bwd(const d3ga_raster_params *prm, const float *means3D, const float *shs,
                                          const float *scales, const float *rotations, const float *cov3D_precomp,
                                          const float *viewmatrix, const float *projmatrix, const float *campos,
                                          const void *geom, const float *acc, float *dL_dmeans3D, float *dL_dmeans2D,
                                          float *dL_dopacity, float *dL_dsh, float *dL_dcolors, float *dL_dcov3D,
                                          float *dL_dscales, float *dL_drots, d3ga_stream_t stream) {
    D3GA_TRY(validate(prm));
    if (prm->P == 0) return D3GA_OK;
    if (!means3D || !viewmatrix || !projmatrix || !campos || !geom || !acc || !dL_dmeans3D) return D3GA_E_NULL;
    if (dL_dsh && !shs) return D3GA_E_NULL;
    if (shs && !dL_dsh && !dL_dcolors) return D3GA_E_NULL;
    if ((dL_dscales != nullptr) != (dL_drots != nullptr)) return D3GA_E_CONFIG;
    if (dL_dscales && (!scales || !rotations)) return D3GA_E_NULL;
    if (!cov3D_precomp && !(scales && rotations)) return D3GA_E_NULL;
    hipStream_t s = (hipStream_t)stream;
    const int views = n_views_of(prm);
    const bool pva = views > 1 && prm->per_view_appearance;
    if (pva && shs) return D3GA_E_CONFIG;
    const GeomBuf g = carve_geom(const_cast<void *>(geom), (int64_t)prm->P * views);
    const size_t lds = lds_bytes(staged(prm, shs), kShLdsBytes);
    const bool win = is_windowed(prm);
    const int cs = cam_stride(prm);
    const dim3 grid((prm->P + kBlock - 1) / kBlock), block(kBlock);
    const size_t pv = prm->per_view_geometry ? (size_t)prm->P : 0;
    auto launch_view = [&](int v, float *dsh, float *dcol, int accum) {
        const ViewCams<1> c = view_cams<1>(viewmatrix, projmatrix, campos, cs, v, 1);
        const size_t o = (size_t)prm->P * v, og = pv * v;
        hipLaunchKernelGGL(win ? preprocess_bwd_kernel<true> : preprocess_bwd_kernel<false>, grid, block, lds, s, *prm, at(means3D, 3, og),
                           shs, at(scales, 3, og), at(rotations, 4, og), c.vm[0], c.pm[0], c.cp[0], geom_view(g, prm->P, v),
                           acc + D3GA_ACC_STRIDE * o, dL_dmeans3D + 3 * og, at(dL_dmeans2D, 3, o), dL_dopacity, dsh, dcol,
                           at(dL_dcov3D, 6, og), at(dL_dscales, 3, og), at(dL_drots, 4, og), at(cov3D_precomp, 6, og), accum);
    };
    if (views == 1) {
        launch_view(0, dL_dsh, dL_dcolors, 0);
        return check_launch(s, prm->debug);
    }
    if (shs ? (dL_dsh != nullptr && leaves_dcol(prm, shs)) : true) {
        for (int v0 = 0; v0 < views; v0 += kMaxGroup) {
            const int kv = views - v0 < kMaxGroup ? views - v0 : kMaxGroup;
            const size_t o = (size_t)prm->P * v0, og = pv * v0, oa = pva ? o : 0;
            hipLaunchKernelGGL(win ? preprocess_bwd_views_kernel<true> : preprocess_bwd_views_kernel<false>, grid, block, lds, s, *prm, kv,
                               at(means3D, 3, og), shs != nullptr, at(scales, 3, og), at(rotations, 4, og), at(cov3D_precomp, 6, og),
                               view_cams<kMaxGroup>(viewmatrix, projmatrix, campos, cs, v0, kv), geom_view(g, prm->P, v0),
                               acc + D3GA_ACC_STRIDE * o, dL_dmeans3D + 3 * og, at(dL_dmeans2D, 3, o), at(dL_dopacity, 1, oa), dL_dsh,
                               at(dL_dcolors, 3, oa), at(dL_dcov3D, 6, og), at(dL_dscales, 3, og), at(dL_drots, 4, og), v0 > 0, pv, pva);
        }
        return check_launch(s, prm->debug);
    }
    if (pva) return D3GA_E_CONFIG;
    if (shs && !dL_dcolors) return D3GA_E_NULL;
    if (prm->factor_rows != 0 && prm->factor_rows < prm->P) return D3GA_E_SIZE;
    const size_t fr = prm->factor_rows > 0 ? (size_t)prm->factor_rows : (size_t)prm->P;
    for (int v = 0; v < views; ++v) launch_view(v, nullptr, shs ? dL_dcolors + 3 * fr * v : dL_dcolors, v > 0 ? (pv ? 1 : 3) : 0);
    D3GA_TRY(check_launch(s, prm->debug));
    if (shs && dL_dsh) {
        hipLaunchKernelGGL(sh_grad_from_views_kernel, grid, block, lds_bytes(sh_staged(prm->M), kShLdsBytes), s, prm->P, prm->M,
                           prm->sh_degree, views, means3D, (int64_t)(3 * pv), dL_dcolors, (int64_t)(3 * fr), campos, (int64_t)cs, 1.0f, dL_dsh);
        return check_launch(s, prm->debug);
    }
    return D3GA_OK;
}

extern "C" int d3ga_sh_grad_from_views(int32_t P, int32_t M, int32_t sh_degree, int32_t n_views, const float *means3D,
                                       const float *g_views, int64_t g_stride, const float *campos_views,
                                       int64_t campos_stride, float scale, float *dL_dsh, d3ga_stream_t stream) {
    if (P < 0 || M < 1 || M > 16 || n_views < 0) return D3GA_E_SIZE;
    if (sh_degree < 0 || sh_degree > 3 || (sh_degree + 1) * (sh_degree + 1) > M) return D3GA_E_CONFIG;
    if (P == 0) return D3GA_OK;
    if (!means3D || !dL_dsh || (n_views > 0 && (!g_views || !campos_views))) return D3GA_E_NULL;
    hipStream_t s = (hipStream_t)stream;
    hipLaunchKernelGGL(sh_grad_from_views_kernel, dim3((P + kBlock - 1) / kBlock), dim3(kBlock), lds_bytes(sh_staged(M), kShLdsBytes), s, P, M, sh_degree,
                       n_views, means3D, (int64_t)0, g_views, g_stride, campos_views, campos_stride, scale, dL_dsh);
    return check_launch(s, 0);
}

extern "C" int d3ga_raster_mark_visible(int32_t P, const float *means3D, const float *viewmatrix, uint8_t *visible,
                                        d3ga_stream_t stream) {
    if (P < 0) return D3GA_E_SIZE;
    if (P == 0) return D3GA_OK;
    if (!means3D || !viewmatrix || !visible) return D3GA_E_NULL;
    hipLaunchKernelGGL(mark_visible_kernel, dim3((P + kBlock - 1) / kBlock), dim3(kBlock), 0, (hipStream_t)stream, P,
                       means3D, viewmatrix, visible);
    return check_launch((hipStream_t)stream, 0);
}
```

Before: 2668.

## Reserve per-wave tile offsets in preprocess so scatter skips global cursor atomics

Result: faster. 2702, median of 6 (+1.3%).

```diff
diff --git a/d3ga_amd/csrc/d3ga_internal.h b/d3ga_amd/csrc/d3ga_internal.h
--- a/d3ga_amd/csrc/d3ga_internal.h
+++ b/d3ga_amd/csrc/d3ga_internal.h
@@ -52,6 +52,8 @@
 struct BinBuf {
     uint32_t *counters;
     uint32_t *tile_count;
+    uint32_t *tile_count2;
+    uint32_t *vis_part;
     uint32_t *tile_start;
     uint32_t *tile_cursor;
     uint64_t *keys;
@@ -61,8 +63,10 @@
     uint32_t *mid_tiles;
     uint32_t *tile_order;
 };
+constexpr int kVisParts = 32, kVisStride = 32;
+constexpr int kUnresvWord = 1;
 static inline int64_t bin_bytes(int64_t tiles, int64_t dcap) {
-    return 256 + align256(4 * tiles) + align256(4 * (tiles + 1)) + align256(4 * tiles) + align256(8 * dcap) +
+    return 256 + 2 * align256(4 * tiles) + 4 * kVisParts * kVisStride + align256(4 * (tiles + 1)) + align256(4 * tiles) + align256(8 * dcap) +
            align256(4 * dcap) + 4 * align256(4 * tiles);
 }
 static inline BinBuf carve_bin(void *base, int64_t tiles, int64_t dcap) {
@@ -70,6 +74,8 @@
     BinBuf b;
     b.counters = (uint32_t *)p;    p += 256;
     b.tile_count = (uint32_t *)p;  p += align256(4 * tiles);
+    b.tile_count2 = (uint32_t *)p; p += align256(4 * tiles);
+    b.vis_part = (uint32_t *)p;    p += 4 * kVisParts * kVisStride;
     b.tile_start = (uint32_t *)p;  p += align256(4 * (tiles + 1));
     b.tile_cursor = (uint32_t *)p; p += align256(4 * tiles);
     b.keys = (uint64_t *)p;        p += align256(8 * dcap);
@@ -100,12 +106,18 @@
     return i;
 }
 
-constexpr int kWinTiles = 4096;
+constexpr int kResvStride = 512;
+constexpr int kResvHdr = 4;
+constexpr int kResvTiles = kResvStride - kResvHdr;
+constexpr int kResvSlots = (kResvTiles + 63) / 64;
+static inline int64_t resv_waves(int64_t P) { return (kBlock / 64) * ((P + kBlock - 1) / kBlock); }
+static inline int64_t resv_bytes(int64_t P, int64_t views) { return align256(4 * kResvStride * resv_waves(P) * views); }
 
 struct TileWindow {
     int x0, y0, w, h;
+    __device__ __forceinline__ bool empty() const { return w <= 0 || h <= 0; }
+    __device__ __forceinline__ bool fits() const { return w <= kResvTiles && h <= kResvTiles && w * h <= kResvTiles; }
     __device__ __forceinline__ int area() const { return w * h; }
-    __device__ __forceinline__ bool fits() const { return w * h <= kWinTiles; }
     __device__ __forceinline__ int tile_of(int k, int gx, float inv_w) const {
         const int r = (int)(((float)k + 0.5f) * inv_w);
         return (y0 + r) * gx + x0 + (k - r * w);
@@ -113,25 +125,18 @@
 };
 
 #ifdef __HIPCC__
-__device__ __forceinline__ TileWindow block_tile_window(int *s_box, bool visible, int rx0, int ry0, int rx1, int ry1) {
-    if (threadIdx.x == 0) { s_box[0] = 0x7fffffff; s_box[1] = 0x7fffffff; s_box[2] = 0; s_box[3] = 0; }
-    __syncthreads();
+__device__ __forceinline__ TileWindow wave_tile_window(bool visible, int rx0, int ry0, int rx1, int ry1) {
     int bx0 = visible ? rx0 : 0x7fffffff, by0 = visible ? ry0 : 0x7fffffff, bx1 = visible ? rx1 : 0, by1 = visible ? ry1 : 0;
 #pragma unroll
     for (int off = 1; off < 64; off <<= 1) {
         bx0 = min(bx0, __shfl_xor(bx0, off)); by0 = min(by0, __shfl_xor(by0, off));
         bx1 = max(bx1, __shfl_xor(bx1, off)); by1 = max(by1, __shfl_xor(by1, off));
     }
-    if ((threadIdx.x & 63) == 0 && bx1 > 0) {
-        atomicMin(&s_box[0], bx0); atomicMin(&s_box[1], by0);
-        atomicMax(&s_box[2], bx1); atomicMax(&s_box[3], by1);
-    }
-    __syncthreads();
     TileWindow win;
-    win.x0 = s_box[0]; win.y0 = s_box[1];
-    win.w = s_box[2] > s_box[0] ? s_box[2] - s_box[0] : 0;
-    win.h = s_box[3] > s_box[1] ? s_box[3] - s_box[1] : 0;
-    if (win.w == 0 || win.h == 0) { win.w = 0; win.h = 0; }
+    win.x0 = bx0; win.y0 = by0;
+    win.w = bx1 > bx0 ? bx1 - bx0 : 0;
+    win.h = by1 > by0 ? by1 - by0 : 0;
+    if (win.w == 0 || win.h == 0) { win.x0 = 0; win.y0 = 0; win.w = 0; win.h = 0; }
     return win;
 }
 #endif
@@ -144,6 +149,9 @@
 static inline int grid_y(const d3ga_raster_params *prm) { return tiles_y(prm->H) + (is_windowed(prm) ? 1 : 0); }
 static inline int4 *win_table(void *binning, int64_t tiles, int64_t dcap) { return (int4 *)((char *)binning + bin_bytes(tiles, dcap)); }
 static inline int64_t win_table_bytes(int64_t views) { return align256(16 * views); }
+static inline uint32_t *resv_records(void *binning, int64_t tiles, int64_t dcap, int64_t views, bool windowed) {
+    return (uint32_t *)((char *)binning + bin_bytes(tiles, dcap) + (windowed ? win_table_bytes(views) : 0));
+}
 
 static inline int check_launch(hipStream_t s, int debug) {
     hipError_t e = hipGetLastError();
diff --git a/d3ga_amd/csrc/raster_api.hip b/d3ga_amd/csrc/raster_api.hip
--- a/d3ga_amd/csrc/raster_api.hip
+++ b/d3ga_amd/csrc/raster_api.hip
@@ -58,7 +58,7 @@
     if ((int64_t)tiles_y(H) * k > 65535 || (int64_t)P * k >= (1ll << 31)) return D3GA_E_SIZE;
     const int64_t tiles = (int64_t)tiles_x(W) * tiles_y(H) * k, cap = d_capacity > 0 ? d_capacity : 1;
     sizes[0] = geom_bytes(P > 0 ? P * k : 1);
-    sizes[1] = bin_bytes(tiles, cap);
+    sizes[1] = bin_bytes(tiles, cap) + resv_bytes(P, k);
     sizes[2] = forward_only ? 2 * align256(4 * (int64_t)W * H * k) : img_bytes(W, H, tiles, cap, k);
     return D3GA_OK;
 }
@@ -72,7 +72,7 @@
     if (gy * k > 65535 || gx > 65535 || (int64_t)P * k >= (1ll << 31)) return D3GA_E_SIZE;
     const int64_t tiles = gx * gy * k, cap = d_capacity > 0 ? d_capacity : 1;
     sizes[0] = geom_bytes(P > 0 ? P * k : 1);
-    sizes[1] = bin_bytes(tiles, cap) + win_table_bytes(k);
+    sizes[1] = bin_bytes(tiles, cap) + win_table_bytes(k) + resv_bytes(P, k);
     sizes[2] = forward_only ? 2 * align256(4 * (int64_t)W * H * k) : img_bytes(W, H, tiles, cap, k);
     return D3GA_OK;
 }
diff --git a/d3ga_amd/csrc/raster_bin.hip b/d3ga_amd/csrc/raster_bin.hip
--- a/d3ga_amd/csrc/raster_bin.hip
+++ b/d3ga_amd/csrc/raster_bin.hip
@@ -6,8 +6,8 @@
 
 constexpr int kScanBlock = 1024;
 
-__device__ __forceinline__ void tile_scan_body(int tiles, const uint32_t *__restrict__ count,
-                                               uint32_t *__restrict__ start, uint32_t *__restrict__ cursor,
+__device__ __forceinline__ void tile_scan_body(int tiles, const uint32_t *__restrict__ count, const uint32_t *__restrict__ count2,
+                                               const uint32_t *__restrict__ vis_part, uint32_t *__restrict__ start, uint32_t *__restrict__ cursor,
                                                uint32_t *__restrict__ counters, uint64_t dcap,
                                                uint32_t *__restrict__ big_tiles, uint32_t *__restrict__ huge_tiles,
                                                uint32_t *__restrict__ mid_tiles, uint32_t n_small, uint32_t n_mid,
@@ -17,18 +17,26 @@
     __shared__ uint32_t s_max;
     const int tid = threadIdx.x, lane = tid & 63, wave = tid >> 6;
     if (tid == 0) s_max = 0;
+    const bool unresv = vis_part[kUnresvWord] != 0u;
+    uint32_t visible = wave == 0 && lane < kVisParts ? vis_part[lane * kVisStride] : 0u;
     uint32_t carry = 0, mx = 0;
     int par = 0;
     for (int c0 = 0; c0 < tiles; c0 += kChunk, par ^= 1) {
         const int t0 = c0 + kPer * tid;
-        uint32_t c[kPer];
+        uint32_t c[kPer], u[kPer];
         if (t0 + kPer <= tiles) {
             const uint4 lo = reinterpret_cast<const uint4 *>(count + t0)[0], hi = reinterpret_cast<const uint4 *>(count + t0)[1];
+            uint4 lo2 = make_uint4(0u, 0u, 0u, 0u), hi2 = lo2;
+            if (unresv) { lo2 = reinterpret_cast<const uint4 *>(count2 + t0)[0]; hi2 = reinterpret_cast<const uint4 *>(count2 + t0)[1]; }
             c[0] = lo.x; c[1] = lo.y; c[2] = lo.z; c[3] = lo.w; c[4] = hi.x; c[5] = hi.y; c[6] = hi.z; c[7] = hi.w;
+            u[0] = lo2.x; u[1] = lo2.y; u[2] = lo2.z; u[3] = lo2.w; u[4] = hi2.x; u[5] = hi2.y; u[6] = hi2.z; u[7] = hi2.w;
         } else {
 #pragma unroll
-            for (int k = 0; k < kPer; ++k) c[k] = t0 + k < tiles ? count[t0 + k] : 0u;
-        }
+            for (int k = 0; k < kPer; ++k) { c[k] = t0 + k < tiles ? count[t0 + k] : 0u; u[k] = unresv && t0 + k < tiles ? count2[t0 + k] : 0u; }
+        }
+        uint32_t any2 = 0;
+#pragma unroll
+        for (int k = 0; k < kPer; ++k) { any2 |= u[k]; c[k] += u[k]; }
         uint32_t sum = 0;
 #pragma unroll
         for (int k = 0; k < kPer; ++k) { sum += c[k]; mx = max(mx, c[k]); }
@@ -80,16 +88,23 @@
         if (t0 + kPer <= tiles) {
             const uint4 lo = make_uint4(e[0], e[1], e[2], e[3]), hi = make_uint4(e[4], e[5], e[6], e[7]);
             reinterpret_cast<uint4 *>(start + t0)[0] = lo; reinterpret_cast<uint4 *>(start + t0)[1] = hi;
-            reinterpret_cast<uint4 *>(cursor + t0)[0] = lo; reinterpret_cast<uint4 *>(cursor + t0)[1] = hi;
         } else {
 #pragma unroll
             for (int k = 0; k < kPer; ++k)
-                if (t0 + k < tiles) { start[t0 + k] = e[k]; cursor[t0 + k] = e[k]; }
+                if (t0 + k < tiles) start[t0 + k] = e[k];
+        }
+        if (any2) {
+#pragma unroll
+            for (int k = 0; k < kPer; ++k)
+                if (t0 + k < tiles && u[k]) cursor[t0 + k] = e[k] + (c[k] - u[k]);
         }
         carry += total;
     }
 #pragma unroll
-    for (int off = 1; off < 64; off <<= 1) mx = max(mx, (uint32_t)__shfl_xor((int)mx, off));
+    for (int off = 1; off < 64; off <<= 1) {
+        mx = max(mx, (uint32_t)__shfl_xor((int)mx, off));
+        visible += (uint32_t)__shfl_xor((int)visible, off);
+    }
     if (lane == 0) atomicMax(&s_max, mx);
     __syncthreads();
     if (tid == 0) {
@@ -97,15 +112,17 @@
         counters[D3GA_CNT_D] = carry;
         counters[D3GA_CNT_OVERFLOW] = (uint64_t)carry > dcap ? 1u : 0u;
         counters[D3GA_CNT_MAXTILE] = s_max;
-    }
-}
-
-__device__ __forceinline__ void tile_order_body(int tiles, const uint32_t *__restrict__ count,
-                                                uint32_t *__restrict__ order, uint32_t *__restrict__ counters) {
+        counters[D3GA_CNT_VISIBLE] = visible;
+    }
+}
+
+__device__ __forceinline__ void tile_order_body(int tiles, const uint32_t *__restrict__ count, const uint32_t *__restrict__ count2,
+                                                const uint32_t *__restrict__ vis_part, uint32_t *__restrict__ order, uint32_t *__restrict__ counters) {
     __shared__ uint32_t s_hist[256];
     __shared__ uint32_t s_zero;
     const int tid = threadIdx.x, lane = tid & 63;
     constexpr int kPer = 8;
+    const bool unresv = vis_part[kUnresvWord] != 0u;
     if (tid < 256) s_hist[tid] = 0;
     if (tid == 0) s_zero = 0;
     __syncthreads();
@@ -115,7 +132,7 @@
 #pragma unroll
         for (int k = 0; k < kPer; ++k) {
             const int t = c0 + k * kScanBlock + tid;
-            c[k] = t < tiles ? count[t] : 0xffffffffu;
+            c[k] = t < tiles ? count[t] + (unresv ? count2[t] : 0u) : 0xffffffffu;
         }
 #pragma unroll
         for (int k = 0; k < kPer; ++k) {
@@ -151,7 +168,7 @@
 #pragma unroll
                 for (int k = 0; k < kPer; ++k) {
                     const int t = c1 + k * kScanBlock + tid;
-                    c[k] = t < tiles ? count[t] : 0xffffffffu;
+                    c[k] = t < tiles ? count[t] + (unresv ? count2[t] : 0u) : 0xffffffffu;
                 }
             }
 #pragma unroll
@@ -170,6 +187,8 @@
 }
 
 __global__ __launch_bounds__(kScanBlock) void tile_scan_order_kernel(int tiles, const uint32_t *__restrict__ count,
+                                                                     const uint32_t *__restrict__ count2,
+                                                                     const uint32_t *__restrict__ vis_part,
                                                                      uint32_t *__restrict__ start,
                                                                      uint32_t *__restrict__ cursor,
                                                                      uint32_t *__restrict__ counters, uint64_t dcap,
@@ -178,47 +197,54 @@
                                                                      uint32_t *__restrict__ mid_tiles, uint32_t n_small,
                                                                      uint32_t n_mid, uint32_t n_large,
                                                                      uint32_t *__restrict__ order) {
-    if (blockIdx.x == 0) tile_scan_body(tiles, count, start, cursor, counters, dcap, big_tiles, huge_tiles, mid_tiles, n_small, n_mid, n_large);
-    else tile_order_body(tiles, count, order, counters);
+    if (blockIdx.x == 0) tile_scan_body(tiles, count, count2, vis_part, start, cursor, counters, dcap, big_tiles, huge_tiles, mid_tiles, n_small, n_mid, n_large);
+    else tile_order_body(tiles, count, count2, vis_part, order, counters);
 }
 
 __global__ __launch_bounds__(kBlock) void tile_scatter_kernel(int P, int gx, const uint2 *__restrict__ rect,
                                                               const float *__restrict__ depth,
+                                                              const uint32_t *__restrict__ start,
+                                                              const uint32_t *__restrict__ resv,
                                                               uint32_t *__restrict__ cursor, uint64_t *__restrict__ keys,
                                                               uint64_t dcap) {
-    __shared__ int s_box[4];
-    __shared__ uint32_t s_cnt[kWinTiles];
-    const int tid = threadIdx.x;
+    __shared__ uint32_t s_cur[kBlock / 64][kResvTiles];
+    const int tid = threadIdx.x, lane = tid & 63, wave = tid >> 6;
     const int i = blockIdx.x * kBlock + tid;
+    if (i - lane >= P) return;
+    const size_t j = (size_t)blockIdx.y * P + i;
+    const uint32_t *rec = resv + ((size_t)blockIdx.y * gridDim.x * (kBlock / 64) + blockIdx.x * (kBlock / 64) + wave) * kResvStride;
+    const uint2 box = *reinterpret_cast<const uint2 *>(rec);
+    uint32_t base[kResvSlots];
+    base[0] = rec[kResvHdr + lane];
     int x0 = 0, y0 = 0, x1 = 0, y1 = 0;
     uint64_t key = 0;
     if (i < P) {
-        const uint2 rc = rect[i];
+        const uint2 rc = rect[j];
         x0 = rc.x & 0xffffu; y0 = rc.x >> 16; x1 = rc.y & 0xffffu; y1 = rc.y >> 16;
-        key = ((uint64_t)__float_as_uint(depth[i]) << 32) | (uint32_t)i;
+        key = ((uint64_t)__float_as_uint(depth[j]) << 32) | (uint32_t)j;
     }
     const bool visible = x1 > x0 && y1 > y0;
-    const TileWindow win = block_tile_window(s_box, visible, x0, y0, x1, y1);
-    const int area = win.area();
-    if (area == 0) return;
+    TileWindow win;
+    win.x0 = (int)(box.x & 0xffffu); win.y0 = (int)(box.x >> 16); win.w = (int)(box.y & 0xffffu); win.h = (int)(box.y >> 16);
+    if (win.empty()) return;
     if (win.fits()) {
-        for (int k = tid; k < area; k += kBlock) s_cnt[k] = 0;
-        __syncthreads();
-        if (visible)
-            for (int ty = y0; ty < y1; ++ty)
-                for (int tx = x0; tx < x1; ++tx) atomicAdd(&s_cnt[(ty - win.y0) * win.w + (tx - win.x0)], 1u);
-        __syncthreads();
+        const int area = win.area();
+        uint32_t *cur = s_cur[wave];
         const float inv_w = 1.0f / (float)win.w;
-        for (int k = tid; k < area; k += kBlock) {
-            const uint32_t c = s_cnt[k];
-            if (c) s_cnt[k] = atomicAdd(&cursor[win.tile_of(k, gx, inv_w)], c);
-        }
-        __syncthreads();
+#pragma unroll
+        for (int q = 1; q < kResvSlots; ++q) base[q] = lane + 64 * q < area ? rec[kResvHdr + lane + 64 * q] : 0u;
+#pragma unroll
+        for (int q = 0; q < kResvSlots; ++q) {
+            const int k = lane + 64 * q;
+            if (k < area) cur[k] = start[win.tile_of(k, gx, inv_w)] + base[q];
+        }
+        __builtin_amdgcn_wave_barrier();
         if (visible)
             for (int ty = y0; ty < y1; ++ty)
                 for (int tx = x0; tx < x1; ++tx) {
                     const int l = (ty - win.y0) * win.w + (tx - win.x0);
-                    const uint32_t pos = atomicAdd(&s_cnt[l], 1u);
+                    if ((unsigned)l >= (unsigned)area) continue;
+                    const uint32_t pos = atomicAdd(&cur[l], 1u);
                     if (pos < dcap) keys[pos] = key;
                 }
     } else if (visible) {
@@ -511,13 +537,14 @@
     const int64_t P = (int64_t)prm->P * views;
     BinBuf bin = carve_bin(binning, tiles, d_capacity);
     GeomBuf g = carve_geom(geom, P);
-    hipLaunchKernelGGL(tile_scan_order_kernel, dim3(2), dim3(kScanBlock), 0, s, tiles, bin.tile_count, bin.tile_start,
+    hipLaunchKernelGGL(tile_scan_order_kernel, dim3(2), dim3(kScanBlock), 0, s, tiles, bin.tile_count, bin.tile_count2, bin.vis_part, bin.tile_start,
                        bin.tile_cursor, bin.counters, (uint64_t)d_capacity, bin.big_tiles, bin.huge_tiles, bin.mid_tiles,
                        (uint32_t)kSortSmall, (uint32_t)kSortMid, (uint32_t)kSortLarge, bin.tile_order);
     D3GA_TRY(check_launch(s, prm->debug));
     if (P == 0 || d_capacity == 0) return D3GA_OK;
-    hipLaunchKernelGGL(tile_scatter_kernel, dim3((unsigned)((P + kBlock - 1) / kBlock)), dim3(kBlock), 0, s, (int)P, gx, g.rect,
-                       g.depth, bin.tile_cursor, bin.keys, (uint64_t)d_capacity);
+    hipLaunchKernelGGL(tile_scatter_kernel, dim3((unsigned)((prm->P + kBlock - 1) / kBlock), (unsigned)views), dim3(kBlock), 0, s, prm->P,
+                       gx, g.rect, g.depth, bin.tile_start, resv_records(binning, tiles, d_capacity, views, is_windowed(prm)),
+                       bin.tile_cursor, bin.keys, (uint64_t)d_capacity);
     D3GA_TRY(check_launch(s, prm->debug));
     {
         static std::atomic<int> resident[64] = {};
diff --git a/d3ga_amd/csrc/raster_pre.hip b/d3ga_amd/csrc/raster_pre.hip
--- a/d3ga_amd/csrc/raster_pre.hip
+++ b/d3ga_amd/csrc/raster_pre.hip
@@ -99,8 +99,12 @@
 }
 
 struct TileRect { bool visible; int r0, r1, r2, r3; };
-__device__ __forceinline__ TileRect write_geom_records(const GeomBuf &geom, int i, const PreOut &o, bool keep_cov, int tile_row0,
-                                                       int32_t *__restrict__ radii, bool want_j, const ShColJ &cj) {
+__device__ __forceinline__ TileRect view_tile_rect(const PreOut &o, int tile_row0) {
+    const Splat &sp = o.sp;
+    return TileRect{sp.visible, sp.rect[0], sp.rect[1] + tile_row0, sp.rect[2], sp.rect[3] + tile_row0};
+}
+__device__ __forceinline__ void write_geom_records(const GeomBuf &geom, int i, const PreOut &o, bool keep_cov, int tile_row0,
+                                                   int32_t *__restrict__ radii, bool want_j, const ShColJ &cj) {
     const Splat &sp = o.sp;
     if (keep_cov) {
 #pragma unroll
@@ -119,7 +123,6 @@
     geom.rgb_invd[i] = make_float4(o.rgb[0], o.rgb[1], o.rgb[2], sp.visible ? 1.0f / sp.depth : 0.f);
     geom.clamped[i] = o.clampmask;
     if (want_j) dcol_store(geom.dcol, geom.dcol_stride, i, cj);
-    return TileRect{sp.visible, sp.rect[0], sp.rect[1] + tile_row0, sp.rect[2], sp.rect[3] + tile_row0};
 }
 
 __device__ __forceinline__ PreOut window_clip(PreOut o, int x0, int y0, int gx, int gy) {
@@ -137,38 +140,59 @@
     table[v] = make_int4(c.ox, c.oy, c.W, c.H);
 }
 
-__device__ __forceinline__ void tile_histogram(int *s_box, uint32_t *s_cnt, const TileRect &t, int gx, uint32_t *__restrict__ tile_count,
-                                               uint32_t *__restrict__ counters) {
-    const int tid = threadIdx.x;
-    const TileWindow win = block_tile_window(s_box, t.visible, t.r0, t.r1, t.r2, t.r3);
-    const int nvis = __syncthreads_count(t.visible);
-    if (tid == 0 && nvis) atomicAdd(&counters[D3GA_CNT_VISIBLE], (uint32_t)nvis);
-    const int area = win.area();
-    if (area == 0) return;
-    if (win.fits()) {
-        for (int k = tid; k < area; k += kBlock) s_cnt[k] = 0;
-        __syncthreads();
+struct TileResv { TileWindow win; uint32_t base[kResvSlots]; };
+__device__ __forceinline__ TileResv tile_reserve_issue(uint32_t *s_win, const TileRect &t, int gx, uint32_t *__restrict__ tile_count,
+                                                       uint32_t *__restrict__ tile_count2, uint32_t *__restrict__ vis_part) {
+    const int lane = threadIdx.x & 63;
+    TileResv r;
+    r.win = wave_tile_window(t.visible, t.r0, t.r1, t.r2, t.r3);
+#pragma unroll
+    for (int j = 0; j < kResvSlots; ++j) r.base[j] = 0u;
+    const unsigned long long vis = __ballot(t.visible);
+    if (lane == 0 && vis) atomicAdd(&vis_part[((blockIdx.x * (kBlock / 64) + (threadIdx.x >> 6)) % kVisParts) * kVisStride], (uint32_t)__popcll(vis));
+    if (r.win.empty()) return r;
+    if (r.win.fits()) {
+        const int area = r.win.area();
+        __builtin_amdgcn_wave_barrier();
+#pragma unroll
+        for (int j = 0; j < kResvSlots; ++j)
+            if (lane + 64 * j < area) s_win[lane + 64 * j] = 0u;
+        __builtin_amdgcn_wave_barrier();
         if (t.visible)
             for (int ty = t.r1; ty < t.r3; ++ty)
-                for (int tx = t.r0; tx < t.r2; ++tx) atomicAdd(&s_cnt[(ty - win.y0) * win.w + (tx - win.x0)], 1u);
-        __syncthreads();
-        const float inv_w = 1.0f / (float)win.w;
-        for (int k = tid; k < area; k += kBlock) {
-            const uint32_t c = s_cnt[k];
-            if (c) atomicAdd(&tile_count[win.tile_of(k, gx, inv_w)], c);
+                for (int tx = t.r0; tx < t.r2; ++tx) atomicAdd(&s_win[(ty - r.win.y0) * r.win.w + (tx - r.win.x0)], 1u);
+        __builtin_amdgcn_wave_barrier();
+        const float inv_w = 1.0f / (float)r.win.w;
+#pragma unroll
+        for (int j = 0; j < kResvSlots; ++j) {
+            const int k = lane + 64 * j;
+            const uint32_t c = k < area ? s_win[k] : 0u;
+            if (c) r.base[j] = atomicAdd(&tile_count[r.win.tile_of(k, gx, inv_w)], c);
         }
-    } else if (t.visible) {
-        for (int ty = t.r1; ty < t.r3; ++ty)
-            for (int tx = t.r0; tx < t.r2; ++tx) atomicAdd(&tile_count[ty * gx + tx], 1u);
-    }
+    } else {
+        if (lane == 0) atomicOr(&vis_part[kUnresvWord], 1u);
+        if (t.visible)
+            for (int ty = t.r1; ty < t.r3; ++ty)
+                for (int tx = t.r0; tx < t.r2; ++tx) atomicAdd(&tile_count2[ty * gx + tx], 1u);
+    }
+    return r;
+}
+__device__ __forceinline__ void tile_reserve_store(const TileResv &r, uint32_t *__restrict__ rec) {
+    const int lane = threadIdx.x & 63;
+    if (lane == 0)
+        *reinterpret_cast<uint4 *>(rec) = make_uint4((uint32_t)r.win.x0 | ((uint32_t)r.win.y0 << 16), (uint32_t)r.win.w | ((uint32_t)r.win.h << 16), 0u, 0u);
+    if (r.win.empty() || !r.win.fits()) return;
+    const int area = r.win.area();
+#pragma unroll
+    for (int j = 0; j < kResvSlots; ++j)
+        if (lane + 64 * j < area) rec[kResvHdr + lane + 64 * j] = r.base[j];
 }
 
 template <bool WIN>
-__device__ __forceinline__ TileRect preprocess_view(const d3ga_raster_params &prm, const ViewCam &cam, int i, const float *means3D,
+__device__ __forceinline__ PreOut preprocess_view(const d3ga_raster_params &prm, const ViewCam &cam, int i, const float *means3D,
                                                     const float *sh_row, bool staged, const ShColJ &cj, bool pre, const float (&pc6)[6],
                                                     float pop, const float *colors_precomp, const float *opacities, const float *scales,
-                                                    const float *rotations, const float *cov3D_precomp, const GeomBuf &geom,
-                                                    int tile_row0, int32_t *radii, bool want_j, int gx, int gy) {
+                                                    const float *rotations, const float *cov3D_precomp, int gx, int gy) {
     PreLoaded pl;
     pl.has_sh = staged; pl.has_c6 = pre;
     pl.sh[0] = cj.a0; pl.sh[1] = cj.a1; pl.sh[2] = cj.a2;
@@ -177,7 +201,7 @@
     pl.op = pop;
     PreOut o = preprocess_one(prm, cam, i, means3D, sh_row, colors_precomp, opacities, scales, rotations, cov3D_precomp, pl);
     if constexpr (WIN) o = window_clip(o, cam.ox / kTile, cam.oy / kTile, gx, gy);
-    return write_geom_records(geom, i, o, !cov3D_precomp, tile_row0, radii, want_j, cj);
+    return o;
 }
 
 template <bool WANT_J, bool WIN>
@@ -186,18 +210,18 @@
     const float *__restrict__ colors_precomp, const float *__restrict__ opacities, const float *__restrict__ scales,
     const float *__restrict__ rotations, const float *__restrict__ cov3D_precomp, const float *__restrict__ viewmatrix,
     const float *__restrict__ projmatrix, const float *__restrict__ campos, GeomBuf geom,
-    uint32_t *__restrict__ tile_count, uint32_t *__restrict__ counters, int32_t *__restrict__ radii,
+    uint32_t *__restrict__ tile_count, uint32_t *__restrict__ tile_count2, uint32_t *__restrict__ vis_part,
+    uint32_t *__restrict__ resv , int32_t *__restrict__ radii,
     int tile_row0 ) {
     const ViewCam cam = view_cam(prm, viewmatrix, projmatrix, campos, WIN);
     const int gx = (prm.W + kTile - 1) / kTile + (WIN ? 1 : 0), gy = (prm.H + kTile - 1) / kTile + 1;
     extern __shared__ __attribute__((aligned(16))) char smem[];
-    __shared__ int s_box[4];
     float *s_sh = reinterpret_cast<float *>(smem);
-    uint32_t *s_cnt = reinterpret_cast<uint32_t *>(smem);
-    const int tid = threadIdx.x;
+    const int tid = threadIdx.x, wave = tid >> 6;
     const int i = blockIdx.x * kBlock + tid;
     const int M3 = 3 * prm.M;
     const bool staged = shs != nullptr && sh_staged(prm.M);
+    uint32_t *s_win = reinterpret_cast<uint32_t *>(smem) + wave * (staged ? kShHalfSlab : kResvStride);
     float pc6[6] = {0.f, 0.f, 0.f, 0.f, 0.f, 0.f}, pop = 0.f;
     const bool pre = staged && cov3D_precomp != nullptr;
     if (pre && i < prm.P) {
@@ -210,17 +234,19 @@
     if (staged) {
         staged_sh_colour<WANT_J>(prm, means3D, shs, campos, s_sh, acc, cj);
         if (!WANT_J) { cj.a0 = acc[0]; cj.a1 = acc[1]; cj.a2 = acc[2]; }
-        __syncthreads();
     }
     TileRect tr = {false, 0, 0, 0, 0};
+    PreOut o = {};
     if (i < prm.P) {
-        tr = staged ? preprocess_view<WIN>(prm, cam, i, means3D, nullptr, true, cj, pre, pc6, pop, colors_precomp, opacities, scales,
-                                           rotations, cov3D_precomp, geom, tile_row0, radii, WANT_J, gx, gy)
-                    : preprocess_view<WIN>(prm, cam, i, means3D, shs ? shs + (size_t)M3 * i : nullptr, false, cj, false, pc6, pop,
-                                           colors_precomp, opacities, scales, rotations, cov3D_precomp, geom, tile_row0, radii,
-                                           WANT_J, gx, gy);
-    }
-    tile_histogram(s_box, s_cnt, tr, gx, tile_count, counters);
+        o = staged ? preprocess_view<WIN>(prm, cam, i, means3D, nullptr, true, cj, pre, pc6, pop, colors_precomp, opacities, scales,
+                                          rotations, cov3D_precomp, gx, gy)
+                   : preprocess_view<WIN>(prm, cam, i, means3D, shs ? shs + (size_t)M3 * i : nullptr, false, cj, false, pc6, pop,
+                                          colors_precomp, opacities, scales, rotations, cov3D_precomp, gx, gy);
+        tr = view_tile_rect(o, tile_row0);
+    }
+    const TileResv rs = tile_reserve_issue(s_win, tr, gx, tile_count, tile_count2, vis_part);
+    if (i < prm.P) write_geom_records(geom, i, o, !cov3D_precomp, tile_row0, radii, WANT_J, cj);
+    tile_reserve_store(rs, resv + (size_t)(blockIdx.x * (kBlock / 64) + wave) * kResvStride);
 }
 
 template <bool WANT_J, int KV>
@@ -280,14 +306,15 @@
     d3ga_raster_params prm, const float *__restrict__ means3D, const float *__restrict__ shs,
     const float *__restrict__ colors_precomp, const float *__restrict__ opacities, const float *__restrict__ scales,
     const float *__restrict__ rotations, const float *__restrict__ cov3D_precomp, ViewCams<KV> cams, GeomBuf geom ,
-    uint32_t *__restrict__ tile_count, uint32_t *__restrict__ counters, int32_t *__restrict__ radii ,
+    uint32_t *__restrict__ tile_count, uint32_t *__restrict__ tile_count2, uint32_t *__restrict__ vis_part,
+    uint32_t *__restrict__ resv , int32_t *__restrict__ radii ,
     int tile_row0, int gyv, size_t pv ) {
     extern __shared__ __attribute__((aligned(16))) char smem[];
-    __shared__ int s_box[4];
     float *s_sh = reinterpret_cast<float *>(smem);
-    uint32_t *s_cnt = reinterpret_cast<uint32_t *>(smem);
-    const int tid = threadIdx.x;
+    const int tid = threadIdx.x, wave = tid >> 6;
     const int i = blockIdx.x * kBlock + tid;
+    uint32_t *s_win = reinterpret_cast<uint32_t *>(smem) + wave * kShHalfSlab;
+    const size_t wpv = (size_t)gridDim.x * (kBlock / 64);
     float pc6[6] = {0.f, 0.f, 0.f, 0.f, 0.f, 0.f}, pop = 0.f;
     const bool pre = cov3D_precomp != nullptr && pv == 0;
     if (pre && i < prm.P) {
@@ -302,16 +329,19 @@
     const int gx = (prm.W + kTile - 1) / kTile;
 #pragma unroll
     for (int v = 0; v < KV; ++v) {
-        __syncthreads();
         TileRect tr = {false, 0, 0, 0, 0};
+        PreOut o = {};
         if (i < prm.P) {
             const size_t og = pv * v;
-            tr = preprocess_view<false>(prm, view_cam(prm, cams.vm[v], cams.pm[v], cams.cp[v], false), i, means3D + 3 * og, nullptr, true,
-                                        cj[v], pre, pc6, pop, colors_precomp, opacities, scales ? scales + 3 * og : nullptr,
-                                        rotations ? rotations + 4 * og : nullptr, cov3D_precomp ? cov3D_precomp + 6 * og : nullptr,
-                                        geom_view(geom, prm.P, v), tile_row0 + v * gyv, radii + (size_t)prm.P * v, WANT_J, gx, 0);
+            o = preprocess_view<false>(prm, view_cam(prm, cams.vm[v], cams.pm[v], cams.cp[v], false), i, means3D + 3 * og, nullptr, true,
+                                       cj[v], pre, pc6, pop, colors_precomp, opacities, scales ? scales + 3 * og : nullptr,
+                                       rotations ? rotations + 4 * og : nullptr, cov3D_precomp ? cov3D_precomp + 6 * og : nullptr, gx, 0);
+            tr = view_tile_rect(o, tile_row0 + v * gyv);
         }
-        tile_histogram(s_box, s_cnt, tr, gx, tile_count, counters);
+        const TileResv rs = tile_reserve_issue(s_win, tr, gx, tile_count, tile_count2, vis_part);
+        if (i < prm.P)
+            write_geom_records(geom_view(geom, prm.P, v), i, o, !cov3D_precomp, tile_row0 + v * gyv, radii + (size_t)prm.P * v, WANT_J, cj[v]);
+        tile_reserve_store(rs, resv + (wpv * v + blockIdx.x * (kBlock / 64) + wave) * kResvStride);
     }
 }
 
@@ -577,7 +607,7 @@
     const int64_t tiles = (int64_t)grid_x(prm) * gyv * views;
     const bool wnd = is_windowed(prm);
     BinBuf bin = carve_bin(binning, tiles, d_capacity);
-    D3GA_HIP(zero_async(bin.counters, 256 + align256(4 * tiles), s));
+    D3GA_HIP(zero_async(bin.counters, 256 + 2 * align256(4 * tiles) + 4 * kVisParts * kVisStride, s));
     if (wnd) hipLaunchKernelGGL(window_table_kernel, dim3((views + 63) / 64), dim3(64), 0, s, *prm, campos, views, win_table(binning, tiles, d_capacity));
     if (prm->P == 0) return D3GA_OK;
     if ((shs != nullptr) == (colors_precomp != nullptr)) return D3GA_E_CONFIG;
@@ -588,7 +618,9 @@
     if (shs && (prm->sh_degree + 1) * (prm->sh_degree + 1) > prm->M) return D3GA_E_CONFIG;
     if (!means3D || !opacities || !radii) return D3GA_E_NULL;
     const GeomBuf g = carve_geom(geom, (int64_t)prm->P * views);
-    const size_t lds = lds_bytes(staged(prm, shs), kShHalfLdsBytes, (size_t)kWinTiles * 4);
+    const size_t lds = lds_bytes(staged(prm, shs), kShHalfLdsBytes, (size_t)(kBlock / 64) * kResvStride * 4);
+    uint32_t *const resv = resv_records(binning, tiles, d_capacity, views, wnd);
+    const size_t resv_view = (size_t)resv_waves(prm->P) * kResvStride;
     const bool want_j = leaves_dcol(prm, shs);
     const int cs = cam_stride(prm);
     const size_t pv = (views > 1 && prm->per_view_geometry) ? (size_t)prm->P : 0;
@@ -602,7 +634,8 @@
         hipLaunchKernelGGL((want_j ? preprocess_views_kernel<true, KV> : preprocess_views_kernel<false, KV>), grid, block, lds, s, *prm,
                            at(means3D, 3, og), shs, colors_precomp, opacities, at(scales, 3, og), at(rotations, 4, og),
                            at(cov3D_precomp, 6, og), view_cams<KV>(viewmatrix, projmatrix, campos, cs, v0, KV), geom_view(g, prm->P, v0),
-                           bin.tile_count, bin.counters, radii + (size_t)prm->P * v0, v0 * gyv, gyv, pv);
+                           bin.tile_count, bin.tile_count2, bin.vis_part, resv + resv_view * v0, radii + (size_t)prm->P * v0, v0 * gyv,
+                           gyv, pv);
         v0 += KV;
     };
     while (grouped && views - v0 >= 2) {
@@ -618,7 +651,8 @@
         const size_t og = pv * v, oa = pa * v;
         hipLaunchKernelGGL(kernel, grid, block, lds, s, *prm, at(means3D, 3, og), shs, at(colors_precomp, 3, oa), opacities + oa,
                            at(scales, 3, og), at(rotations, 4, og), at(cov3D_precomp, 6, og), c.vm[0], c.pm[0], c.cp[0],
-                           geom_view(g, prm->P, v), bin.tile_count, bin.counters, radii + (size_t)prm->P * v, v * gyv);
+                           geom_view(g, prm->P, v), bin.tile_count, bin.tile_count2, bin.vis_part, resv + resv_view * v,
+                           radii + (size_t)prm->P * v, v * gyv);
     }
     return check_launch(s, prm->debug & 0xff);
 }
```
